# opteroncx/MoePhoto

Measured on AMD Instinct MI355X. Metric: megapixels/sec (input), 1080p 4x SR (Net4x a4), 256-px tiles with overlap, higher is better.
Workload: dtype fp16; 1 GPU; BASELINE configs[1]: 1 frame(s) 1920x1080 RGB -> 7680x4320, model a4 (Net4x, synthetic weights in zoo format), crop 256 pad 5 align 8 -> 40 tiles/frame, fp16 I/O, fp16 MFMA operands + fp32 accumulate; tiles_per_frame=40, parallelism=single GPU, precision=mixed, exact_blocks=1, input=natural-image-like synthetic frame (tests/golden_defs.natural_image)

## Files before the change

moephoto_amd/csrc/common.h:

```cpp
#pragma once
#include <hip/hip_runtime.h>
#include <stdint.h>

typedef _Float16 half_t;
typedef __attribute__((ext_vector_type(2))) _Float16 half2_t;
typedef __attribute__((ext_vector_type(4))) _Float16 half4_t;
typedef __attribute__((ext_vector_type(8))) _Float16 half8_t;
typedef __attribute__((ext_vector_type(4))) float float4_t;
typedef __attribute__((ext_vector_type(16))) float float16_t;

constexpr int kCB = 64;
constexpr int kTileW = 32;
constexpr int kTileH = 8;
constexpr int kFragBytes = 1024;

struct ConvArgs {
    const half_t* in;
    half_t* out;
    const half_t* res;
    const half_t* wpk;
    const float* bias;
    const float* bias_img;
    const half_t* zero;
    half_t* trash;
    half_t* out_lo;
    const half_t* in_lo;
    int plane_w;
    const half_t* side16;
    const float* tail1_w;
    float* tail1_out;
    const half_t* res_lo;
    float* acc32;
    int acc_mode;
    long long w_batch_stride;
    int B, H, W;
    int in_cs, out_cs;
    int r;
    int nchunks;
    int G;
    int px, py;
    float slope;
    float scale;
    const half_t* tail_w;
    float* tplanes;
    int tail_form;
    int tail_split;
    int dbg;
    float* pool; int pool_slabs;
};

struct ConvForm {
    int B = 0, H = 0, W = 0, in_cs = 64, out_cs = 64, r = 1, nchunks = 1, G = 1, py = 1;
    float slope = 1.f, scale = 1.f;
    int acc_mode = 0, dbg = 0, tail_form = 0, tail_split = 0, pool_slabs = 0;
    bool res = false, res_lo = false, in_lo = false, out_lo = false, side16 = false, tail = false, tail1 = false, pool = false, plane_w = false;
};
inline ConvForm conv_form(const ConvArgs& a)
{
    ConvForm c;
    c.B = a.B; c.H = a.H; c.W = a.W; c.in_cs = a.in_cs; c.out_cs = a.out_cs; c.r = a.r; c.nchunks = a.nchunks; c.G = a.G; c.py = a.py;
    c.slope = a.slope; c.scale = a.scale; c.acc_mode = a.acc_mode; c.dbg = a.dbg; c.tail_form = a.tail_form; c.tail_split = a.tail_split; c.pool_slabs = a.pool_slabs;
    c.res = a.res != nullptr; c.res_lo = a.res_lo != nullptr; c.in_lo = a.in_lo != nullptr; c.out_lo = a.out_lo != nullptr; c.side16 = a.side16 != nullptr;
    c.tail = a.tplanes != nullptr; c.tail1 = a.tail1_w != nullptr; c.pool = a.pool != nullptr; c.plane_w = a.plane_w != 0;
    return c;
}

struct TailSumLayout { unsigned S, RA, CA, CO, total; int py, px; };
__host__ __device__ inline TailSumLayout tailsum_layout(int B, int H, int W)
{
    TailSumLayout l;
    l.py = (H + kTileH - 1) / kTileH; l.px = (W + kTileW - 1) / kTileW;
    auto up = [](unsigned long long n) { return (unsigned)((n + 63) / 64 * 64); };
    l.S = 0;
    l.RA = l.S + up(16ull * B * H * W);
    l.CA = l.RA + up(8ull * B * l.py * W);
    l.CO = l.CA + up(8ull * B * H * l.px);
    l.total = l.CO + up(4ull * B * l.py * l.px);
    return l;
}
inline bool tailsum_fits(int B, int H, int W)
{
    const unsigned long long el = 16ull * B * H * W + 8ull * B * ((H + kTileH - 1) / kTileH) * W + 8ull * B * H * ((W + kTileW - 1) / kTileW) + 4ull * B * ((H + kTileH - 1) / kTileH) * ((W + kTileW - 1) / kTileW) + 4 * 64;
    return el * 4 < (1ull << 32) - (1ull << 17);
}

struct Conv1x1Args {
    const half_t* in_hi; const half_t* in_lo;
    half_t* out_hi; half_t* out_lo;
    const half_t* w_hi; const half_t* w_lo;
    const float* bias;
    const float* tail_w; float* tail_out;
    float slope;
    int B, H, W, r, nchunks, out_cs;
    int nks;
};
struct Conv1x1Form { int B, H, W, r, nchunks, out_cs; float slope; bool x3, tail, out_lo; };
bool conv1x1_applicable(const Conv1x1Form& a, int max_groups);
bool launch_conv1x1(const Conv1x1Args& a, int max_groups, hipStream_t s);
hipError_t conv1x1_init();

struct Conv1x1F2Args {
    const half_t* in_hi; const half_t* in_lo;
    const half_t* wa_hi; const half_t* wa_lo;
    const half_t* wb_hi; const half_t* wb_lo;
    const float* bias_a; const float* bias_b;
    const float* tail_w; float* tail_out;
    float slope_a, slope_b;
    int B, H, W;
};
bool conv1x1_f2_applicable(int B, int H, int W, float slope_a, float slope_b, int max_groups);
bool launch_conv1x1_f2(const Conv1x1F2Args& a, int max_groups, hipStream_t s);
hipError_t conv1x1_f2_init();

void launch_conv_mfma(const ConvArgs& a, int taps, int nseg, hipStream_t s);
int conv_mfma_max_groups();
hipError_t conv_mfma_init();
bool conv3x3_sp_applicable(const ConvForm& c);
bool launch_conv3x3_sp(const ConvArgs& a, hipStream_t s);
hipError_t conv3x3_sp_init();
bool conv3x3_rw_applicable(const ConvForm& c);
bool launch_conv3x3_rw(const ConvArgs& a, hipStream_t s);
hipError_t conv3x3_rw_init();

struct Ps4Args {
    const half_t* in;
    const half_t* wpk;
    const float* bias;
    const half_t* tail_w;
    half_t* out;
    float* plane;
    float* apron;
    float slope;
    int B, H, W;
    int split;
};
bool launch_conv3x3_ps4(const Ps4Args& a, int max_groups, hipStream_t s);
bool ps4_applicable(int B, int H, int W);
inline bool ps4_tail_applicable(int B, int H, int W, float slope) { return slope < 1.f && ps4_applicable(B, H, W); }
bool ps4_store_applicable(int B, int H, int W, float slope);
size_t ps4_plane_bytes(int B, int H, int W);
size_t ps4_apron_bytes(int B, int H, int W);
hipError_t conv3x3_ps4_init();
struct TailAddArgs {
    const float* p0; const float* p1;
    const float* a0; const float* a1;
    void* y; int y_dtype; const long long* y_off;
    int B, H, W, px;
    int vec_ok;
};
void launch_tailadd(const TailAddArgs& a, hipStream_t s);

struct Ps9Args {
    const half_t* in;
    const half_t* wpk;
    const float* bias;
    const half_t* tail_w;
    float* plane;
    float* apron;
    float slope;
    int B, H, W;
    int split;
    int xcd_map;
};
bool launch_conv3x3_ps9(const Ps9Args& a, int max_groups, hipStream_t s);
bool ps9_applicable(int B, int H, int W);
inline bool ps9_tail_applicable(int B, int H, int W, float slope) { return slope < 1.f && ps9_applicable(B, H, W); }
size_t ps9_plane_bytes(int B, int H, int W);
size_t ps9_apron_bytes(int B, int H, int W);
hipError_t conv3x3_ps9_init();
struct TailAdd3Args {
    const float* p0; const float* p1;
    const float* a0; const float* a1;
    void* y; int y_dtype; const long long* y_off;
    int B, H, W, px;
    int vec_ok;
};
void launch_tailadd3(const TailAdd3Args& a, hipStream_t s);

struct ArsbArgs {
    const half_t* x_hi; const half_t* x_lo;
    half_t* y_hi; half_t* y_lo;
    const half_t* w1; const half_t* w2;
    const half_t* zero;
    float slope;
    int B, H, W;
    int px, py;
    int cin;
    int drop_lo;
    unsigned long long* trace;
};
bool arsb32c_applicable(int B, int H, int W, float slope, bool x_lo, bool y_lo, int cin);
bool launch_arsb32c(ArsbArgs a, int max_groups, hipStream_t s);
hipError_t arsb32c_init();

struct ConvX3Args {
    const half_t* in_hi; const half_t* in_lo;
    half_t* out_hi; half_t* out_lo;
    const half_t* res_hi; const half_t* res_lo;
    const half_t* w_hi; const half_t* w_lo;
    const half_t* zero;
    float slope;
    int B, H, W;
    int px, py;
    float* pool; int pool_slabs;
    const float* gate;
    const half_t* wq_hi16; const unsigned char* wq_hi8; const unsigned char* wq_lo8;
    int in8, out8;
};
struct ConvX3Form {
    int B = 0, H = 0, W = 0, pool_slabs = 0;
    float slope = 1.f;
    bool res = false, res_lo = false, pool = false, gate = false, in8 = false, out8 = false;
};
inline ConvX3Form conv_x3_form(const ConvX3Args& a)
{
    ConvX3Form c;
    c.B = a.B; c.H = a.H; c.W = a.W; c.pool_slabs = a.pool_slabs; c.slope = a.slope;
    c.res = a.res_hi != nullptr; c.res_lo = a.res_lo != nullptr; c.pool = a.pool != nullptr; c.gate = a.gate != nullptr; c.in8 = a.in8 != 0; c.out8 = a.out8 != 0;
    return c;
}
bool conv64_x3_applicable(const ConvX3Form& c, int max_groups);
bool launch_conv64_x3(ConvX3Args a, int max_groups, hipStream_t s);
hipError_t conv64_x3_init();
bool conv64_q8_applicable(const ConvX3Form& c);
bool launch_conv64_q8(ConvX3Args a, int max_groups, hipStream_t s);
hipError_t conv64_q8_init();
bool conv64_sq_applicable(const ConvX3Form& c, int max_groups);
bool launch_conv64_sq(ConvX3Args a, int max_groups, hipStream_t s);
hipError_t conv64_sq_init();
bool conv64_s_applicable(const ConvForm& c);
bool launch_conv64_s(const ConvArgs& a, int max_groups, hipStream_t s);
hipError_t conv64_s_init();
struct ArsbSqArgs {
    const half_t* x_hi; const unsigned char* x_lo8;
    half_t* y_hi; void* y_lo;
    const half_t* w16[2]; const unsigned char* wh8[2]; const unsigned char* wl8[2];
    float slope;
    int B, H, W, out8;
};
bool arsb_sq_applicable(int B, int H, int W, float slope);
bool launch_arsb_sq(const ArsbSqArgs& a, int max_groups, hipStream_t s);
hipError_t arsb_sq_init();

inline int pooled_groups(long long P, long long items, int max_groups)
{
    long long G = 1;
    if (P <= max_groups) G = P * (max_groups / P);
    else for (long long d = max_groups; d >= 1; --d) if (P % d == 0) { G = d; break; }
    return (int)(G < items ? G : items);
}
inline bool pooled_groups_ok(long long P, long long items, int max_groups)
{
    const long long full = items < max_groups ? items : max_groups;
    return 2ll * pooled_groups(P, items, max_groups) >= full;
}

struct DirectConvArgs {
    const half_t* in; half_t* out; const half_t* res;
    const float* w;
    const float* bias;
    long long w_batch_stride;
    int B, H, W, in_cs, out_cs, cin, cout, k, r;
    float slope, scale;
};
void launch_conv_direct(const DirectConvArgs& a, hipStream_t s);

struct StemArgs {
    const void* x; int x_dtype;
    const long long* x_off;
    long long sB, sH, sW;
    const float* w;
    float slope;
    half_t* out;
    half_t* out_lo;
    int B, H, W, taps;
    int out_lo8;
    const float* w2; half_t* out2; half_t* out2_lo;
};
void launch_stem(const StemArgs& a, hipStream_t s);

struct TailArgs {
    const half_t* in0; const half_t* in1;
    const half_t* w0; const half_t* w1;
    const half_t* in0_lo; const half_t* in1_lo;
    const half_t* w0_lo; const half_t* w1_lo;
    int in1_lo8;
    const void* skip; int skip_dtype;
    const long long* skip_off; long long skip_sB, skip_sH, skip_sW;
    void* y; int y_dtype;
    const long long* y_off;
    int B, H, W, taps;
};
void launch_tail(const TailArgs& a, hipStream_t s);

struct TapSumArgs {
    const float* t0; const float* t1;
    void* y; int y_dtype; const long long* y_off;
    int B, H, W;
    int r;
    int form;
    int vec_ok;
};
void launch_tapsum(const TapSumArgs& a, hipStream_t s);

struct Tail1SumArgs {
    const float* p0; const float* p1;
    int nparts;
    void* y; int y_dtype; const long long* y_off;
    int B, H, W;
    const float* lut; int r; const void* x; const long long* x_off; long long sB, sH, sW;
    int vec_ok;
};
void launch_tail1sum(const Tail1SumArgs& a, hipStream_t s);

void launch_pool_partial(const half_t* in, const half_t* in_lo, float* partial, int B, long long HW, int C, int nslab, hipStream_t s);

struct SednSeArgs {
    const float* partial; int nslab; long long HW;
    const float* w_down;
    const float* w_up;
    const float* trans_pk32;
    half_t* trans_out;
    half_t* trans_out_lo;
    int B, nfrag;
};
void launch_sedn_se(const SednSeArgs& a, hipStream_t s);

struct SednFuseArgs {
    const half_t* x;
    float* partial;
    const float* pooled; int pooled_slabs;
    int pooled_count;
    int nslab, B, H, W;
    const float* w256t;
    const float* w256;
    const float* wt;
    const float* w_down;
    const float* w_up;
    float* gate;
    half_t* weff;
};
void launch_sedn_fuse(const SednFuseArgs& a, hipStream_t s);

struct FrmArgs {
    const float* partial; int nslab; long long HW;
    const float* w0; const float* b0;
    const float* w2; const float* b2;
    const half_t* t; const half_t* x; half_t* out;
    const half_t* t_lo; const half_t* x_lo; half_t* out_lo;
    float* gate;
    int B;
};
void launch_frm(const FrmArgs& a, hipStream_t s);
struct FrmPreArgs {
    const half_t* m; const half_t* m_lo;
    const float* partial; int nslab;
    const float* c2t;
    const float* w0; const float* b0;
    const float* w2; const float* b2;
    float* gate;
    int B, H, W;
};
void launch_frm_pre(const FrmPreArgs& a, hipStream_t s);

struct StitchArgs {
    const float* tiles; const long long* tile_off;
    const int* row_first; const int* row_cnt;
    const int* col_first; const int* col_cnt;
    const int* row_tab; const int* col_tab;
    const float* ramp;
    void* out; int out_dtype;
    int C, out_h, out_w, step_w;
    int row_lo;
    int y0, rows;
};
void launch_stitch(const StitchArgs& a, hipStream_t s);
bool launch_stitch_out(const StitchArgs& a, int canvas_dtype, float quant, hipStream_t s);
struct StitchMix {
    const void* inp; long long sC, sH, sW;
    const void* alpha; long long aH, aW;
    float sf, tf; int blend;
    float quant;
    int inp_vec, alpha_vec;
    long long once_from; int q_once;
};
bool launch_stitch_mix(const StitchArgs& a, StitchMix m, int canvas_dtype, hipStream_t s);
struct YuvEdge {
    int ky[3], ku[3], kv[3];
    unsigned mul_y, base_y; int mul_c, base_c;
    int depth, f16;
};
void launch_stitch_yuv(const StitchArgs& a, const YuvEdge& y, hipStream_t s);
void launch_to_output_yuv(const void* src, int src_dtype, int H, int W, const YuvEdge& y, void* dst, hipStream_t s);

struct BlendTileArgs {
    const void* r; void* canvas; const void* ramp;
    long long r_sC, r_sH, c_sC, c_sH;
    int C, rh, rw;
    int top_sc, left_sc;
    int r0, c0;
    int lt_h, lt_w;
};
void launch_blend_tile(const BlendTileArgs& a, bool f16, hipStream_t s);

struct SymArgs {
    const void* src; void* dst;
    long long sC, sH, sW;
    int C, Hd, Wd;
    int nR, nC, flipR, flipC;
    int src_vec;
    int div; float inv;
};
void launch_sym(SymArgs a, bool f16, bool fold, bool tr, hipStream_t s);

struct WireRec {
    long long tile_off, wire_off;
    int C, th, tw;
    int ra0, ra1, rb0, rb1;
    int ca0, ca1, cb0, cb1;
    int pad_;
};
long long wire_rec_words(const WireRec& r);
void launch_wire(bool pack, float* tiles, unsigned* wire, const WireRec* recs, int n, long long max_elems, hipStream_t s);

void launch_to_float(const void* src, int src_dtype, float inv_or_div, bool divide, int H, int W, int C, void* dst, int dst_dtype, hipStream_t s);
void launch_to_output(const void* src, int src_dtype, int H, int W, int C, float quant, void* dst, int dst_dtype, hipStream_t s);
void launch_resize(const void* src, void* dst, int dtype, int C, int H, int W, int h, int w, int mode, hipStream_t s);
void launch_maxabsdiff(const float* a, const float* b, long long n, unsigned* out, hipStream_t s);
void launch_nhwc_to_nchw_f32(const half_t* in, const half_t* in_lo, float* out, int B, int H, int W, int cs, int C, hipStream_t s);
```

moephoto_amd/csrc/forward.cpp:

```cpp
#include "net.h"

using namespace moe;

namespace moe {

const char* kernel_name(ConvKernel k)
{
    static const char* const names[] = {"no kernel", "conv_direct", "conv1x1", "conv_mfma", "conv3x3_sp", "conv3x3_rw", "conv3x3_ps4 (store form)", "conv3x3_sp (hi + lo residual)",
                                        "conv_mfma (three products)", "conv64_x3", "conv64_q8", "conv64_sq", "conv3x3_sp (three launches)", "conv_mfma (fp32 side buffer)"};
    return names[(int)k];
}

static bool fast_layer(const moe_net& n, const ConvLayer& L) { return L.taps == 9 && L.nseg == 1 && !L.per_plane && n.opt.conv_impl == 2; }

ConvForm Fwd::form(const ConvLayer& L, int H, int W) const
{
    ConvForm c;
    c.B = B; c.H = H; c.W = W; c.in_cs = 64 * L.nseg; c.out_cs = L.r > 1 ? 64 : 64 * L.nchunks; c.r = L.r; c.nchunks = L.nchunks;
    c.py = (H + kTileH - 1) / kTileH;
    const long long items = (long long)B * ((W + kTileW - 1) / kTileW) * c.py;
    const int per_xcd = groups / 8;
    int G = per_xcd >= L.nchunks ? 8 * (per_xcd / L.nchunks) : groups / L.nchunks;
    if (G < 1) G = 1;
    if (G > items) G = (int)items;
    c.G = G;
    c.slope = L.slope; c.scale = L.scale; c.dbg = n.opt.dbg;
    return c;
}

ConvRoute Fwd::route(const std::string& key, const Act& in, const Act& out, const Act* res, int H, int W, const ConvExtra& e) const
{
    ConvRoute r;
    auto take = [&r](ConvKernel k) { r.kernel = k; return r; };
    auto refuse = [&r]() { r.kernel = ConvKernel::none; r.done.ok = false; return r; };
    const ConvLayer& L = n.convs[n.conv_index.at(key)];
    const bool x3 = this->x3 || e.exact;
    const bool res_lo = res && res->has_lo;
    const bool any8 = in.lo8 || out.lo8 || (res && res->lo8);
    if (any8 && !(x3 && use_q8() && q8_capable(L) && !direct)) return refuse();
    if (e.fuse_tail1) r.done.tail1_parts = 2;
    ConvForm& c = r.form;
    c = form(L, H, W);
    if (direct) return take(ConvKernel::direct);
    const int px = (W + kTileW - 1) / kTileW;
    c.res = res != nullptr; c.tail1 = e.fuse_tail1;
    c.tail = e.fuse_tail; c.tail_form = e.fuse_tail ? tail_form : 0; c.tail_split = (e.fuse_tail && mixed && tail_split_for(key)) ? 1 : 0;
    if (e.pool && !x3 && L.r == 1 && L.nchunks == 1 && !res && pooled_groups_ok((long long)c.py, (long long)B * c.py, groups)) {
        c.pool = true; c.pool_slabs = e.pool_slabs;
        c.G = pooled_groups((long long)c.py, (long long)B * c.py, groups);
    }
    const bool fast = fast_layer(n, L);
    if (e.fuse_tail && !(fast && !x3)) return refuse();
    if (n.opt.conv1x1 && L.taps == 1 && L.nseg == 1 && !L.per_plane && !res && L.scale == 1.f && !e.fuse_tail && n.opt.conv_impl == 2 && (!x3 || (in.has_lo && L.has_x3)) &&
        conv1x1_applicable(Conv1x1Form{B, H, W, L.r, L.nchunks, c.out_cs, L.slope, x3, e.fuse_tail1, x3 && out.has_lo}, groups)) {
        if (e.fuse_tail1) r.done.tail1_parts = 1;
        return take(ConvKernel::conv1x1);
    }
    const bool traced = !x3 && (c.dbg & 64) && fast && key == n.opt.trace_key;
    if (!x3 && !traced && res_lo && out.has_lo) {
        c.acc_mode = 3; c.side16 = true; c.out_lo = true;
        r.done.ok = fast && conv3x3_sp_applicable(c);
        return take(ConvKernel::sp_res_lo);
    }
    if (!x3) {
        if (c.tail && c.tail_form == 1) { r.done.ok = conv3x3_rw_applicable(c); return take(ConvKernel::rw); }
        if (fast && n.opt.up_impl == 1 && !c.tail && !c.pool && c.r == 2 && c.nchunks == 4 && c.in_cs == 64 && !c.res && c.scale == 1.f && !c.dbg && L.has_bias &&
            (long long)B * px * (H / 4) >= 32ll * groups && ps4_store_applicable(B, H, W, L.slope))
            return take(ConvKernel::ps4_store);
        if (fast && n.opt.sp_impl && !c.tail && conv3x3_rw_applicable(c)) { r.done.pooled = c.pool; return take(ConvKernel::rw); }
        if (fast && conv3x3_sp_applicable(c)) return take(ConvKernel::sp);
        if (c.tail) return refuse();
        return take(ConvKernel::mfma);
    }
    if (L.has_x3 && !fast) return take(ConvKernel::mfma_x3);
    if (n.opt.x3_fuse && fast && L.w_arsb_lo && in.has_lo && out.has_lo && (!res || res_lo) && !e.fuse_tail && !L.has_bias) {
        ConvX3Form q;
        q.B = B; q.H = H; q.W = W; q.slope = L.slope; q.res = res != nullptr; q.res_lo = res_lo;
        const long long P = (long long)px * c.py;
        if (e.pool && !res && (L.slope == 1.f || e.pool_act) && pooled_groups_ok(P, (long long)B * P, groups)) { q.pool = true; q.pool_slabs = e.pool_slabs; }
        if (e.gate && res && !use_q8()) q.gate = true;
        r.x3 = q;
        if (use_q8() && L.wq_hi8 && !q.pool && (!res || res->lo8 == in.lo8)) {
            r.x3.in8 = in.lo8; r.x3.out8 = out.lo8;
            if (n.opt.q8_impl == 1 && conv64_sq_applicable(r.x3, groups)) return take(ConvKernel::sq);
            if (conv64_q8_applicable(r.x3)) return take(ConvKernel::q8);
            r.x3 = q;
        }
        if (any8) return refuse();
        if (conv64_x3_applicable(q, groups)) { r.done.pooled = q.pool; r.done.gated = q.gate; return take(ConvKernel::x3); }
    }
    if (fast && L.nchunks <= 16) {
        ConvForm q1 = c; q1.res = res_lo; q1.slope = 1.f; q1.scale = 1.f; q1.tail = false;
        ConvForm q2 = q1; q2.res = true;
        ConvForm q3 = c; q3.acc_mode = 3; q3.side16 = true; q3.out_lo = out.has_lo;
        if (conv3x3_sp_applicable(q1) && conv3x3_sp_applicable(q2) && conv3x3_sp_applicable(q3)) return take(ConvKernel::sp_three);
    }
    if (!acc32_elems) return refuse();
    return take(ConvKernel::acc32);
}

int Fwd::launch(const ConvRoute& r, const std::string& key, const Act& in, const Act& out, const Act* res, const ConvExtra& e)
{
    const ConvLayer& L = n.convs[n.conv_index.at(key)];
    const ConvForm& c = r.form;
    const int H = c.H, W = c.W;
    if (r.kernel == ConvKernel::direct) {
        DirectConvArgs d{};
        d.in = in.hi; d.out = out.hi; d.res = res ? res->hi : nullptr;
        d.w = blob<float>(L.w_plain);
        d.bias = L.has_bias ? blob<float>(L.bias_plain) : nullptr;
        d.w_batch_stride = 0;
        d.B = B; d.H = H; d.W = W; d.in_cs = c.in_cs; d.out_cs = c.out_cs; d.cin = L.cin; d.cout = L.cout; d.k = L.k; d.r = L.r;
        d.slope = L.slope; d.scale = L.scale;
        if (L.per_plane) { d.w = (const float*)e.plane_w; d.w_batch_stride = (long long)L.cout * L.cin; }
        launch_conv_direct(d, s);
        return MOE_OK;
    }
    ConvArgs a{};
    a.in = in.hi; a.out = out.hi; a.res = res ? res->hi : nullptr;
    a.wpk = L.per_plane ? e.plane_w : blob<half_t>(L.w_hi);
    a.bias = L.has_bias ? blob<float>(L.bias) : small<float>("zero_bias");
    a.zero = small<half_t>("zero");
    a.bias_img = blob<float>(L.bias_img);
    a.trash = small<half_t>("trash");
    a.w_batch_stride = L.per_plane ? (long long)L.nchunks * L.nfrag() * 512 : 0;
    a.B = B; a.H = H; a.W = W; a.in_cs = c.in_cs; a.out_cs = c.out_cs; a.r = c.r; a.nchunks = c.nchunks;
    a.px = (W + kTileW - 1) / kTileW; a.py = c.py; a.G = c.G;
    a.slope = c.slope; a.scale = c.scale; a.dbg = c.dbg;
    a.tail_w = e.tail_w; a.tplanes = e.tplanes; a.tail_form = c.tail_form; a.tail_split = c.tail_split;
    a.tail1_w = e.tail1_w; a.tail1_out = e.tail1_out;
    if (c.pool) { a.pool = e.pool_out; a.pool_slabs = c.pool_slabs; }
    const bool x3 = this->x3 || e.exact;
    const bool timed = r.kernel != ConvKernel::mfma_x3 && r.kernel != ConvKernel::sp_three && r.kernel != ConvKernel::acc32;
    const int rec = timed ? prof_begin(key, (x3 ? 3 : 1) * 2.0 * (double)B * H * W * L.cout * L.cin * L.taps) : -1;
    bool ok = true;
    auto single = [&](const ConvArgs& ca) {
        if (r.kernel == ConvKernel::rw) return launch_conv3x3_rw(ca, s);
        if (r.kernel == ConvKernel::sp) return launch_conv3x3_sp(ca, s);
        if (r.kernel == ConvKernel::ps4_store) {
            Ps4Args q{};
            q.in = ca.in; q.wpk = ca.wpk; q.bias = ca.bias; q.out = ca.out; q.slope = ca.slope; q.B = ca.B; q.H = ca.H; q.W = ca.W;
            return launch_conv3x3_ps4(q, groups, s);
        }
        launch_conv_mfma(ca, L.taps, L.nseg, s);
        return true;
    };
    switch (r.kernel) {
    case ConvKernel::conv1x1: {
        Conv1x1Args q{};
        q.in_hi = in.hi; q.in_lo = x3 ? in.lo : nullptr; q.out_hi = out.hi; q.out_lo = x3 ? out.lo : nullptr;
        q.w_hi = blob<half_t>(L.w_hi); q.w_lo = x3 ? blob<half_t>(L.w_lo) : nullptr; q.bias = a.bias;
        q.tail_w = e.tail1_w; q.tail_out = e.tail1_out; q.slope = L.slope;
        q.B = B; q.H = H; q.W = W; q.r = L.r; q.nchunks = L.nchunks; q.out_cs = c.out_cs;
        q.nks = (L.cin <= 48 && n.opt.k48) ? 3 : 4;
        ok = launch_conv1x1(q, groups, s);
        break;
    }
    case ConvKernel::mfma: case ConvKernel::sp: case ConvKernel::rw: case ConvKernel::ps4_store: {
        unsigned long long* tr = nullptr;
        const size_t nb = 8 * 32 * 4 * 16 * 8;
        if (!x3 && (c.dbg & 64) && fast_layer(n, L) && key == n.opt.trace_key && hipMalloc((void**)&tr, nb) == hipSuccess) {
            (void)hipMemsetAsync(tr, 0, nb, s);
            ConvArgs t = a; t.acc32 = (float*)tr;
            ok = single(t);
            std::vector<unsigned long long> host(nb / 8);
            (void)hipStreamSynchronize(s);
            (void)hipMemcpy(host.data(), tr, nb, hipMemcpyDeviceToHost);
            if (FILE* f = fopen("/tmp/moe_trace.bin", "wb")) { fwrite(host.data(), 1, nb, f); fclose(f); }
            (void)hipFree(tr);
        } else
            ok = single(a);
        break;
    }
    case ConvKernel::sp_res_lo: {
        ConvArgs q = a; q.acc_mode = 3; q.side16 = res->lo; q.out_lo = out.lo; q.res_lo = nullptr;
        ok = launch_conv3x3_sp(q, s);
        break;
    }
    case ConvKernel::mfma_x3: {
        ConvArgs f4 = a; f4.wpk = blob<half_t>(L.w_x3); f4.acc_mode = 4; f4.in_lo = in.lo; f4.out_lo = out.lo; f4.res_lo = res ? res->lo : nullptr;
        launch_conv_mfma(f4, 1, 3, s);
        break;
    }
    case ConvKernel::x3: case ConvKernel::q8: case ConvKernel::sq: {
        ConvX3Args q{};
        q.in_hi = in.hi; q.in_lo = in.lo; q.out_hi = out.hi; q.out_lo = out.lo;
        q.res_hi = res ? res->hi : nullptr; q.res_lo = res ? res->lo : nullptr;
        q.w_hi = blob<half_t>(L.w_arsb); q.w_lo = blob<half_t>(L.w_arsb_lo); q.zero = small<half_t>("zero");
        q.slope = L.slope; q.B = B; q.H = H; q.W = W;
        if (r.x3.pool) { q.pool = e.pool_out; q.pool_slabs = e.pool_slabs; }
        if (r.x3.gate) q.gate = e.gate_in;
        if (r.kernel == ConvKernel::x3) { ok = launch_conv64_x3(q, groups, s); break; }
        q.wq_hi16 = blob<half_t>(L.w_hi); q.wq_hi8 = blob<unsigned char>(L.wq_hi8); q.wq_lo8 = blob<unsigned char>(L.wq_lo8);
        q.in8 = r.x3.in8; q.out8 = r.x3.out8;
        ok = r.kernel == ConvKernel::sq ? launch_conv64_sq(q, groups, s) : launch_conv64_q8(q, groups, s);
        break;
    }
    case ConvKernel::sp_three: {
        ConvArgs q1 = a; q1.wpk = blob<half_t>(L.w_lo); q1.out = side16; q1.res = (res && res->has_lo) ? res->lo : nullptr; q1.bias = small<float>("zero_bias");
        q1.bias_img = small<float>("zero_bias_img"); q1.slope = 1.f; q1.scale = 1.f; q1.acc_mode = 0; q1.tail_w = nullptr; q1.tplanes = nullptr;
        ConvArgs q2 = q1; q2.in = in.lo; q2.wpk = blob<half_t>(L.w_hi); q2.res = side16;
        ConvArgs q3 = a; q3.acc_mode = 3; q3.side16 = side16; q3.out_lo = out.lo; q3.res_lo = nullptr;
        ok = launch_conv3x3_sp(q1, s) && launch_conv3x3_sp(q2, s) && launch_conv3x3_sp(q3, s);
        break;
    }
    case ConvKernel::acc32: {
        a.acc32 = acc32;
        ConvArgs p1 = a; p1.wpk = L.per_plane ? e.plane_w_lo : blob<half_t>(L.w_lo); p1.acc_mode = 1; p1.res = nullptr; p1.bias = nullptr;
        launch_conv_mfma(p1, L.taps, L.nseg, s);
        ConvArgs p2 = a; p2.in = in.lo; p2.acc_mode = 2; p2.res = nullptr; p2.bias = nullptr;
        launch_conv_mfma(p2, L.taps, L.nseg, s);
        ConvArgs p3 = a; p3.acc_mode = 3; p3.out_lo = out.lo; p3.res_lo = res ? res->lo : nullptr;
        launch_conv_mfma(p3, L.taps, L.nseg, s);
        break;
    }
    default: ok = false;
    }
    prof_end(rec);
    if (!ok) return fail(MOE_EINVAL, "internal error: layer %s (%d planes of %dx%d) was routed to %s, and that launcher refused it", key.c_str(), B, H, W, kernel_name(r.kernel));
    return MOE_OK;
}

ConvDone Fwd::conv(const std::string& key, const Act& in, const Act& out, const Act* res, int H, int W, const ConvExtra& e)
{
    const ConvRoute r = route(key, in, out, res, H, W, e);
    if (r.done.ok && !dry()) {
        rc = launch(r, key, in, out, res, e);
        if (rc) ar.base = nullptr;
    }
    return r.done;
}

void Fwd::stem(const Act& out, const Act* out2)
{
    if (dry()) return;
    StemArgs a{};
    if (out2) { a.w2 = small<float>("stem.p2"); a.out2 = out2->hi; a.out2_lo = out2->lo; }
    a.x = io.x; a.x_dtype = io.x_dtype; a.x_off = io.x_off; a.sB = io.sB; a.sH = io.sH; a.sW = io.sW;
    a.w = small<float>("stem"); a.slope = n.scalars.at("stem_slope");
    a.out = out.hi; a.out_lo = out.lo; a.out_lo8 = out.lo8; a.B = B; a.H = h; a.W = w; a.taps = (int)n.scalars.at("stem_taps");
    launch_stem(a, s);
}

void Fwd::gate() { if (ctx.gate_event && !dry()) (void)hipStreamWaitEvent(s, ctx.gate_event, 0); }

void Fwd::tail(const Act* r, const Act* u, int H, int W, bool skip)
{
    gate();
    if (dry()) return;
    TailArgs a{};
    a.in0 = r->hi; a.w0 = small<half_t>("tail_r");
    if (u) { a.in1 = u->hi; a.w1 = small<half_t>("tail_u"); }
    if (r->has_lo && (!u || u->has_lo)) {
        a.in0_lo = r->lo; a.w0_lo = small<half_t>("tail_r.lo");
        if (u) { a.in1_lo = u->lo; a.w1_lo = small<half_t>("tail_u.lo"); a.in1_lo8 = u->lo8; }
    }
    if (skip) { a.skip = io.x; a.skip_dtype = io.x_dtype; a.skip_off = io.x_off; a.skip_sB = io.sB; a.skip_sH = io.sH; a.skip_sW = io.sW; }
    a.y = io.y; a.y_dtype = io.y_dtype; a.y_off = io.y_off; a.B = B; a.H = H; a.W = W; a.taps = (int)n.scalars.at("tail_taps");
    launch_tail(a, s);
}

static size_t acc32_need(const moe_net& n, int B, int h, int w)
{
    size_t best = 0;
    long long HW = (long long)h * w;
    if (n.arch == MOE_ARCH_SEDN) return (size_t)B * (size_t)HW * 256;
    int rr = 1;
    best = (size_t)B * (size_t)HW * 64;
    for (int s = 0; s < n.stages; ++s) {
        best = std::max<size_t>(best, (size_t)B * (size_t)HW * rr * rr * 64 * n.r * n.r);
        rr *= n.r;
    }
    return best;
}

int exact_blocks_of(const moe_net& n)
{
    if (n.exact_blocks >= 0) return n.exact_blocks > 6 ? 6 : n.exact_blocks;
    const int env = n.opt.exact_blocks_env;
    if (env >= 0) return env > 6 ? 6 : env;
    if (n.calib_valid && n.calib_blocks >= 0) return n.calib_blocks;
    return default_exact_blocks(n.arch);
}

int default_exact_blocks(int arch)
{
    switch (arch) {
        case MOE_ARCH_NET2X: return 4;
        case MOE_ARCH_NET3X: return 2;
        case MOE_ARCH_NET4X: return 1;
        case MOE_ARCH_NETDN: return 1;
        default: return 0;
    }
}

long long sp_bytes_per_pixel(const moe_net& n)
{
    long long per = 128;
    if (n.arch == MOE_ARCH_SEDN) per = 512;
    if (n.arch == MOE_ARCH_LITE) {
        for (int st = 0; st + 1 < n.stages; ++st) per *= 4;
    }
    if (n.arch == MOE_ARCH_NET2X || n.arch == MOE_ARCH_NET3X || n.arch == MOE_ARCH_NET4X) {
        long long rr = 1;
        for (int st = 0; st < n.stages; ++st) {
            rr *= (long long)n.r * n.r;
            per = std::max(per, st == n.stages - 1 ? 36 * rr : 128 * rr);
        }
    }
    return per;
}

static int run_forward(const moe_net& n, Fwd& f, const FwdIO& io)
{
    const int B = f.B, h = f.h, w = f.w;
    const long long P = (long long)B * h * w;
    f.io = io;
    if (f.x3) {
        f.acc32_elems = acc32_need(n, B, h, w);
        f.acc32 = (float*)f.ar.take(f.acc32_elems * 4);
        f.side16 = (half_t*)f.ar.take(f.acc32_elems * 2 + 4096);
    } else if (f.mixed) {
        f.side16 = (half_t*)f.ar.take((size_t)P * 64 * 2 + 4096);
        bool steep = false;
        for (int i = 1; i <= exact_blocks_of(n); ++i) steep = steep || n.convs[n.conv_index.at("c1_" + std::to_string(i))].slope > 1.f;
        if (steep) { f.acc32_elems = (size_t)P * 64; f.acc32 = (float*)f.ar.take(f.acc32_elems * 4); }
    }
    int rc = MOE_OK;
    switch (n.arch) {
        case MOE_ARCH_SEDN: rc = forward_sedn(n, f); break;
        case MOE_ARCH_LITE: rc = forward_lite(n, f); break;
        default: rc = forward_arsb(n, f);
    }
    return rc ? rc : f.rc;
}

static Fwd make_fwd(const moe_net& n, const FwdCtx& ctx, NetRuntime* rt, hipStream_t s, int B, int h, int w, Arena ar)
{
    Fwd f{n, ctx, rt, s, B, h, w, ar, ctx.groups, n.precision == MOE_PREC_FP16X3, n.precision == MOE_PREC_DEBUG_DIRECT};
    f.mixed = n.precision == MOE_PREC_MIXED;
    return f;
}

static size_t workspace_need(const moe_net& n, const FwdCtx& ctx, int B, int h, int w)
{
    Fwd f = make_fwd(n, ctx, nullptr, nullptr, B, h, w, Arena{});
    run_forward(n, f, FwdIO{});
    return f.ar.off + 4096;
}

static bool plan_matches(const Fwd& f, size_t planned)
{
    if (f.ar.overflow) return false;
    return f.skips_planned_work ? f.ar.off <= planned : f.ar.off == planned;
}

static int forward_dev_chunk(moe_net& n, const FwdIO& io, int B, int h, int w, hipStream_t s, bool y_off_mult8, const FwdCtx& ctx);

static void build_lite_lut_on_device(moe_net& n, hipStream_t s, const FwdCtx& ctx)
{
    const int r = n.scale;
    std::vector<unsigned short> pat(65536);
    for (int i = 0; i < 65536; ++i) pat[(size_t)i] = (unsigned short)i;
    half_t* in = nullptr;
    float* scratch = nullptr;
    int rc = MOE_ENOMEM;
    if (hipMalloc((void**)&in, 65536 * 2) == hipSuccess && hipMalloc((void**)&n.lut, (size_t)65536 * r * r * 4) == hipSuccess && hipMalloc((void**)&scratch, (size_t)65536 * r * r * 4) == hipSuccess &&
        hipMemcpyAsync(in, pat.data(), 65536 * 2, hipMemcpyHostToDevice, s) == hipSuccess && hipStreamSynchronize(s) == hipSuccess) {
        FwdCtx capture = ctx;
        capture.lut_capture = n.lut;
        rc = forward_dev_chunk(n, FwdIO{in, MOE_F16, 65536, 256, 1, nullptr, scratch, MOE_F32, nullptr}, 1, 256, 256, s, true, capture);
        (void)hipStreamSynchronize(s);
    }
    if (in) (void)hipFree(in);
    if (scratch) (void)hipFree(scratch);
    if (rc != MOE_OK) { (void)hipGetLastError(); drop_lut(n); }
    n.lut_state = rc == MOE_OK ? 1 : -1;
}

static void build_lite_lut(moe_net& n, hipStream_t s, const FwdCtx& ctx)
{
    n.lut_state = -1;
    if (n.arch != MOE_ARCH_LITE || !n.opt.lite_lut || n.debug || !n.opt.fuse_tail || n.precision == MOE_PREC_DEBUG_DIRECT) return;
    hipStreamCaptureStatus cs = hipStreamCaptureStatusNone;
    if (hipStreamIsCapturing(s, &cs) != hipSuccess || cs != hipStreamCaptureStatusNone) { (void)hipGetLastError(); n.lut_state = 0; return; }
    int cur = -1;
    if (hipGetDevice(&cur) != hipSuccess || (cur != n.device && hipSetDevice(n.device) != hipSuccess)) { (void)hipGetLastError(); n.lut_state = 0; return; }
    build_lite_lut_on_device(n, s, ctx);
    if (cur != n.device) (void)hipSetDevice(cur);
}

int forward_dev(moe_net& n, const FwdIO& io, int B, int h, int w, hipStream_t s, bool y_off_mult8, const FwdCtx& ctx)
{
    if (!n.finalized) return fail(MOE_ESTATE, "moe_net_forward: net is not finalized (load_state_dict + to(device) first)");
    if (B < 1 || h < 1 || w < 1) return fail(MOE_EINVAL, "moe_net_forward: bad shape B=%d h=%d w=%d", B, h, w);
    if ((io.x_dtype != MOE_F32 && io.x_dtype != MOE_F16) || (io.y_dtype != MOE_F32 && io.y_dtype != MOE_F16))
        return fail(MOE_EINVAL, "moe_net_forward: x/y dtype must be MOE_F32 or MOE_F16");
    const long long bmax = kSpRange / (sp_bytes_per_pixel(n) * (long long)h * w);
    if (bmax < 1)
        return fail(MOE_ENOMEM, "a %dx%d tile exceeds the convolution kernels' addressing range (%lld pixels per plane at most for this net): use a smaller cropsize",
                    h, w, kSpRange / sp_bytes_per_pixel(n));
    if (n.arch == MOE_ARCH_LITE && io.x_dtype == MOE_F16 && n.lut_state == 0 && n.opt.lite_lut) build_lite_lut(n, s, ctx);
    if (B <= bmax) return forward_dev_chunk(n, io, B, h, w, s, y_off_mult8, ctx);
    const size_t xe = io.x_dtype == MOE_F32 ? 4 : 2, ye = io.y_dtype == MOE_F32 ? 4 : 2;
    const long long yplane = (long long)h * n.scale * w * n.scale;
    for (int b0 = 0; b0 < B; b0 += (int)bmax) {
        const int cnt = (int)std::min<long long>(bmax, B - b0);
        FwdIO c = io;
        if (io.x_off) c.x_off += b0; else c.x = (const char*)io.x + (size_t)b0 * io.sB * xe;
        if (io.y_off) c.y_off += b0; else c.y = (char*)io.y + (size_t)b0 * yplane * ye;
        const bool al = y_off_mult8 && (io.y_off || ((size_t)b0 * yplane * ye) % 16 == 0);
        if (int rc = forward_dev_chunk(n, c, cnt, h, w, s, al, ctx)) return rc;
    }
    return MOE_OK;
}

static int forward_dev_chunk(moe_net& n, const FwdIO& io, int B, int h, int w, hipStream_t s, bool y_off_mult8, const FwdCtx& ctx)
{
    int cur = -1;
    HIP_TRY(hipGetDevice(&cur));
    if (cur != n.device) HIP_TRY(hipSetDevice(n.device));
    const size_t need = workspace_need(n, ctx, B, h, w);
    StreamSet& set = *ctx.set;
    if (int rc = set.ws.grow(need, s, "workspace of %zu bytes for %d planes of %dx%d does not fit", need, B, h, w)) return rc;
    const size_t planned = need - 4096;
    Fwd f = make_fwd(n, ctx, &n.rt, s, B, h, w, Arena{(char*)set.ws.p, 0, planned});
    f.y_vec = y_off_mult8 && ((uintptr_t)io.y % 16 == 0);
    int rc = run_forward(n, f, io);
    if (rc) return rc;
    if (!plan_matches(f, planned))
        return fail(MOE_EINVAL, "internal error: the launching pass took %zu bytes of workspace%s, the planning pass %zu (%d planes of %dx%d)", f.ar.off,
                    f.ar.overflow ? " (beyond the plan: the launches behind that point were not issued)" : "", planned, B, h, w);
    hipError_t e = hipGetLastError();
    if (e != hipSuccess) return fail(MOE_EHIP, "kernel launch failed: %s", hipGetErrorString(e));
    return MOE_OK;
}

void free_set(StreamSet& set)
{
    if (set.side) { (void)hipStreamSynchronize(set.side); (void)hipStreamDestroy(set.side); }
    for (hipEvent_t e : {set.ev_fork, set.ev_join}) if (e) (void)hipEventDestroy(e);
    set.ws.release();
    set = StreamSet{};
}

void free_records(NetRuntime& rt)
{
    for (auto& ev : rt.prof_ev) { (void)hipEventDestroy(ev.e0); (void)hipEventDestroy(ev.e1); }
    for (auto& sl : rt.off_ring) {
        if (sl.host) (void)hipHostFree(sl.host);
        if (sl.dev) (void)hipFree(sl.dev);
        if (sl.done) (void)hipEventDestroy(sl.done);
    }
    for (auto& t : rt.taps) if (t.second.dev) (void)hipFree(t.second.dev);
    rt = NetRuntime{};
}

void pipe_destroy(moe_net& n)
{
    for (auto& ps : n.pipe) {
        if (ps.main) { (void)hipStreamSynchronize(ps.main); (void)hipStreamDestroy(ps.main); }
        for (hipEvent_t e : {ps.entry, ps.done}) if (e) (void)hipEventDestroy(e);
        free_set(ps);
        ps = PipeSet{};
    }
    n.pipe_prev_valid = false;
    n.pipe_last_stream = nullptr;
}

static bool overlap_eligible(const moe_net& n, int B, int h, int w)
{
    const bool sr = n.arch == MOE_ARCH_NET2X || n.arch == MOE_ARCH_NET3X || n.arch == MOE_ARCH_NET4X;
    return sr && n.finalized && n.opt.overlap_calls && !n.debug && n.opt.conv_impl == 2 && (n.precision == MOE_PREC_MIXED || n.precision == MOE_PREC_FP16) &&
           (long long)B * h * w <= 4ll * 65536 && n.prof_keys.empty() && n.opt.repeat_key.empty();
}

static int forward_pipelined(moe_net* n, const void* x, int x_dtype, int B, int h, int w, int64_t sB, int64_t sH, int64_t sW, void* y, int y_dtype, hipStream_t s, unsigned flags)
{
    HIP_TRY(hipSetDevice(n->device));
    PipeSet& ps = n->pipe[n->pipe_next];
    PipeSet& prev = n->pipe[n->pipe_next ^ 1];
    if (!ps.main) {
        HIP_TRY(hipStreamCreateWithFlags(&ps.main, hipStreamNonBlocking));
        HIP_TRY(hipEventCreateWithFlags(&ps.entry, hipEventDisableTiming));
        HIP_TRY(hipEventCreateWithFlags(&ps.done, hipEventDisableTiming));
    }
    HIP_TRY(hipEventRecord(ps.entry, s));
    const bool since_prev = (flags & MOE_FWD_INPUT_SINCE_PREV) && n->pipe_prev_valid && n->pipe_last_stream == s && prev.entry;
    HIP_TRY(hipStreamWaitEvent(ps.main, since_prev ? prev.entry : ps.entry, 0));
    n->pipe_next ^= 1;
    const int groups = n->opt.overlap_groups > 0 ? std::max(16, std::min(n->opt.overlap_groups, n->max_groups)) : std::max(16, n->max_groups / 2);
    const FwdCtx ctx{&ps, groups, n->opt.overlap_fork && n->opt.branch_streams, since_prev ? ps.entry : nullptr, nullptr};
    const int rc = forward_dev(*n, FwdIO{x, x_dtype, sB, sH, sW, nullptr, y, y_dtype, nullptr}, B, h, w, ps.main, true, ctx);
    if (hipEventRecord(ps.done, ps.main) != hipSuccess || hipStreamWaitEvent(s, ps.done, 0) != hipSuccess) { (void)hipGetLastError(); (void)hipStreamSynchronize(ps.main); }
    n->pipe_prev_valid = rc == MOE_OK;
    n->pipe_last_stream = s;
    return rc;
}

}

extern "C" {

int moe_net_forward_ex(moe_net* n, const void* x, int x_dtype, int B, int h, int w, int64_t sB, int64_t sH, int64_t sW,
                       const int64_t* x_off, void* y, int y_dtype, const int64_t* y_off, void* stream, unsigned flags)
{
    if (!n || !x || !y) return fail(MOE_EINVAL, "moe_net_forward: NULL argument");
    if (flags & ~(unsigned)MOE_FWD_INPUT_SINCE_PREV) return fail(MOE_EINVAL, "moe_net_forward_ex: unknown flags 0x%x", flags);
    if ((flags & MOE_FWD_INPUT_SINCE_PREV) && !x_off && !y_off && B >= 1 && h >= 1 && w >= 1 && overlap_eligible(*n, B, h, w)) {
        hipStreamCaptureStatus cs = hipStreamCaptureStatusNone;
        if (hipStreamIsCapturing((hipStream_t)stream, &cs) == hipSuccess && cs == hipStreamCaptureStatusNone)
            return forward_pipelined(n, x, x_dtype, B, h, w, sB, sH, sW, y, y_dtype, (hipStream_t)stream, flags);
        (void)hipGetLastError();
    }
    n->pipe_prev_valid = false;
    return moe_net_forward(n, x, x_dtype, B, h, w, sB, sH, sW, x_off, y, y_dtype, y_off, stream);
}

int moe_net_forward(moe_net* n, const void* x, int x_dtype, int B, int h, int w, int64_t sB, int64_t sH, int64_t sW,
                    const int64_t* x_off, void* y, int y_dtype, const int64_t* y_off, void* stream)
{
    if (!n || !x || !y) return fail(MOE_EINVAL, "moe_net_forward: NULL argument");
    hipStream_t s = (hipStream_t)stream;
    long long* xo = nullptr;
    long long* yo = nullptr;
    NetRuntime::OffSlot* slot = nullptr;
    if (x_off || y_off) {
        HIP_TRY(hipSetDevice(n->device >= 0 ? n->device : 0));
        NetRuntime::OffSlot& sl = n->rt.off_ring[n->rt.off_next];
        n->rt.off_next = (n->rt.off_next + 1) % 4;
        if (sl.used) HIP_TRY(hipEventSynchronize(sl.done));
        const size_t need = (size_t)B * 2;
        if (need > sl.cap) {
            if (sl.host) { (void)hipHostFree(sl.host); sl.host = nullptr; }
            if (sl.dev) { (void)hipFree(sl.dev); sl.dev = nullptr; }
            sl.cap = 0;
            const size_t cap = std::max<size_t>(need, 256);
            HIP_TRY(hipHostMalloc((void**)&sl.host, cap * 8, hipHostMallocDefault));
            HIP_TRY(hipMalloc((void**)&sl.dev, cap * 8));
            sl.cap = cap;
        }
        if (!sl.done) HIP_TRY(hipEventCreateWithFlags(&sl.done, hipEventDisableTiming));
        for (int i = 0; i < B; ++i) { sl.host[i] = x_off ? x_off[i] : 0; sl.host[B + i] = y_off ? y_off[i] : 0; }
        HIP_TRY(hipMemcpyAsync(sl.dev, sl.host, need * 8, hipMemcpyHostToDevice, s));
        sl.used = true;
        slot = &sl;
        if (x_off) xo = sl.dev;
        if (y_off) yo = sl.dev + B;
    }
    bool mult8 = true;
    if (y_off) for (int i = 0; i < B; ++i) mult8 = mult8 && (y_off[i] % 8 == 0);
    const int rc = forward_dev(*n, FwdIO{x, x_dtype, sB, sH, sW, xo, y, y_dtype, yo}, B, h, w, s, mult8, own_ctx(*n, &n->set));
    if (slot && hipEventRecord(slot->done, s) != hipSuccess) { (void)hipGetLastError(); (void)hipStreamSynchronize(s); }
    return rc;
}

int64_t moe_net_workspace_bytes(const moe_net* n, int B, int h, int w)
{
    if (!n || B < 1 || h < 1 || w < 1) return fail(MOE_EINVAL, "moe_net_workspace_bytes: bad argument");
    if (!n->finalized) return fail(MOE_ESTATE, "moe_net_workspace_bytes: net is not finalized");
    return (int64_t)workspace_need(*n, own_ctx(*n, nullptr), B, h, w);
}

int moe_net_set_profile(moe_net* n, const char* layer_substrings)
{
    if (!n) return fail(MOE_EINVAL, "moe_net_set_profile: NULL net");
    n->prof_keys.clear();
    std::string all = layer_substrings ? layer_substrings : "";
    size_t pos = 0;
    while (pos <= all.size() && !all.empty()) {
        const size_t c = all.find(',', pos);
        const std::string k = all.substr(pos, c == std::string::npos ? std::string::npos : c - pos);
        if (!k.empty()) n->prof_keys.push_back(k);
        if (c == std::string::npos) break;
        pos = c + 1;
    }
    n->rt.prof_used = 0;
    return MOE_OK;
}

int moe_net_get_profile_at(moe_net* n, int index, double* total_ms, int64_t* launches, double* flops)
{
    if (!n || !total_ms || !launches || !flops) return fail(MOE_EINVAL, "moe_net_get_profile: NULL argument");
    double ms = 0, fl = 0;
    int64_t cnt = 0;
    for (size_t i = 0; i < n->rt.prof_used; ++i) {
        const NetRuntime::ProfRec& r = n->rt.prof_ev[i];
        if (r.key != index) continue;
        HIP_TRY(hipEventSynchronize(r.e1));
        float t = 0.f;
        HIP_TRY(hipEventElapsedTime(&t, r.e0, r.e1));
        ms += t; fl += r.flops; ++cnt;
    }
    *total_ms = ms; *launches = cnt; *flops = fl;
    return MOE_OK;
}

int moe_net_get_profile(moe_net* n, double* total_ms, int64_t* launches, double* flops)
{
    int rc = moe_net_get_profile_at(n, 0, total_ms, launches, flops);
    if (rc == MOE_OK) n->rt.prof_used = 0;
    return rc;
}

int64_t moe_net_max_tile_pixels(const moe_net* n)
{
    if (!n) return fail(MOE_EINVAL, "moe_net_max_tile_pixels: NULL net");
    return (int64_t)(kSpRange / sp_bytes_per_pixel(*n));
}

int moe_net_set_debug(moe_net* n, int enable)
{
    if (!n) return fail(MOE_EINVAL, "moe_net_set_debug: NULL net");
    n->debug = enable != 0;
    return MOE_OK;
}

int64_t moe_net_debug_tap(moe_net* n, const char* tap, float* host, int64_t capacity, int64_t shape[4], void* stream)
{
    if (!n || !tap) return fail(MOE_EINVAL, "moe_net_debug_tap: NULL argument");
    auto it = n->rt.taps.find(tap);
    if (it == n->rt.taps.end() || !it->second.dev) return fail(MOE_EINVAL, "no tap named \"%s\" (enable moe_net_set_debug before the forward)", tap);
    const auto& t = it->second;
    const int64_t nel = t.shape[0] * t.shape[1] * t.shape[2] * t.shape[3];
    if (shape) for (int d = 0; d < 4; ++d) shape[d] = t.shape[d];
    if (!host) return nel;
    if (capacity < nel) return fail(MOE_EINVAL, "moe_net_debug_tap: capacity %lld < %lld", (long long)capacity, (long long)nel);
    HIP_TRY(hipStreamSynchronize((hipStream_t)stream));
    HIP_TRY(hipMemcpy(host, t.dev, (size_t)nel * 4, hipMemcpyDeviceToHost));
    return nel;
}

}
```

moephoto_amd/csrc/forward_arsb.cpp:

```cpp
#include "net.h"

using namespace moe;

namespace {

const ConvLayer* last_up(const moe_net& n, int br)
{
    const auto it = n.conv_index.find(std::string(br == 0 ? "convt_R1" : "u") + ".up" + std::to_string(n.stages - 1));
    return it == n.conv_index.end() ? nullptr : &n.convs[it->second];
}

bool can_fuse_tail(const moe_net& n, const Fwd& f)
{
    const int B = f.B, h = f.h, w = f.w;
    if (!n.opt.fuse_tail || f.x3 || f.direct || n.debug || n.opt.conv_impl != 2 || n.stages < 1) return false;
    if (!(n.arch == MOE_ARCH_NET2X || n.arch == MOE_ARCH_NET3X || n.arch == MOE_ARCH_NET4X)) return false;
    if (sp_bytes_per_pixel(n) * B * h * w > kSpRange) return false;
    int hl = h, wl = w;
    for (int st = 0; st + 1 < n.stages; ++st) { hl *= n.r; wl *= n.r; }
    for (int br = 0; br < 2; ++br) {
        const ConvLayer* L = last_up(n, br);
        if (!L) return false;
        ConvForm c = f.form(*L, hl, wl);
        c.tail = true;
        if (!conv3x3_sp_applicable(c)) return false;
    }
    return true;
}

struct ArsbRun {
    const moe_net& n;
    Fwd& f;
    const int B, h, w;
    bool mixed = false;
    int nx = 0;
    Act A, Bb, Cc;
    bool chain8 = false;
    half_t* lo16x = nullptr;
    bool sr = false, fuse = false, ps4 = false, ps9 = false;
    int H = 0, W = 0;
    Act fin[2];
    float* tp[2] = {nullptr, nullptr};
    float* ps_plane[2] = {nullptr, nullptr};
    float* ps_apron[2] = {nullptr, nullptr};

    void plan_tail_form();
    template <typename Args, typename Launch>
    int ps_stage(int br, const std::string& key, const Act& cur, size_t plane_bytes, size_t apron_bytes, const char* name, Launch launch);
    int run_branch(int br, Act cur);
    int trunk_conv(const std::string& key, const Act& in, const Act& out, const Act* res, bool exact);
    int run_trunk();
    template <typename Args, typename Launch> void tail_add(Launch launch);
    int branch_sum();
    int run();
};

void ArsbRun::plan_tail_form()
{
    sr = n.arch != MOE_ARCH_NETDN;
    fuse = sr && can_fuse_tail(n, f);
    if (sr) {
        int hl = h, wl = w;
        for (int st = 0; st + 1 < n.stages; ++st) { hl *= n.r; wl *= n.r; }
        bool ok = fuse && n.opt.tail_form == 1;
        bool ps4_ok = true;
        bool ps9_ok = true;
        for (int br = 0; br < 2; ++br) {
            const ConvLayer* L = last_up(n, br);
            if (ok) {
                ConvForm c = f.form(*L, hl, wl);
                c.tail = true; c.tail_form = 1;
                ok = conv3x3_rw_applicable(c);
            }
            ps4_ok = ps4_ok && L && ps4_tail_applicable(B, hl, wl, L->slope);
            ps9_ok = ps9_ok && L && ps9_tail_applicable(B, hl, wl, L->slope);
        }
        f.tail_form = ok ? 1 : 0;
        ps4 = ok && n.opt.up_impl == 1 && ps4_ok && (2 * wl) % 8 == 0;
        ps9 = fuse && n.opt.up_impl == 1 && n.r == 3 && f.groups >= 3 && ps9_ok;
    }
}

template <typename Args, typename Launch>
int ArsbRun::ps_stage(int br, const std::string& key, const Act& cur, size_t plane_bytes, size_t apron_bytes, const char* name, Launch launch)
{
    ps_plane[br] = (float*)f.ar.take(plane_bytes + 4096);
    ps_apron[br] = (float*)f.ar.take(apron_bytes + 4096);
    if (!f.dry()) {
        const ConvLayer& L = n.convs[n.conv_index.at(key)];
        Args q{};
        q.in = cur.hi; q.wpk = f.blob<half_t>(L.w_hi); q.bias = L.has_bias ? f.blob<float>(L.bias) : f.small<float>("zero_bias");
        q.tail_w = f.small<half_t>(br == 0 ? "tail_r.frag" : "tail_u.frag");
        q.plane = ps_plane[br]; q.apron = ps_apron[br]; q.slope = L.slope; q.B = B; q.H = H; q.W = W;
        q.split = (f.mixed && f.tail_split_for(key)) ? 1 : 0;
        const int rec = f.prof_begin(key, 2.0 * (double)B * H * W * L.cout * L.cin * L.taps);
        bool done = false;
        for (int rep = f.repeats(key); rep > 0; --rep) done = launch(q, f.groups, f.s);
        f.prof_end(rec);
        if (!done) return fail(MOE_EINVAL, "fused tail kernel (%s) rejected layer %s", name, key.c_str());
    }
    H *= n.r; W *= n.r;
    return (int)MOE_OK;
}

int ArsbRun::run_branch(int br, Act cur)
{
    if (f.mixed) { cur.drop_lo(); cur.lo8 = false; }
    H = h; W = w;
    for (int st = 0; st < n.stages; ++st) {
        const std::string key = std::string(br == 0 ? "convt_R1" : "u") + ".up" + std::to_string(st);
        if (ps4 && st == n.stages - 1) {
            if (int rc = ps_stage<Ps4Args>(br, key, cur, ps4_plane_bytes(B, H, W), ps4_apron_bytes(B, H, W), "ps4", launch_conv3x3_ps4)) return rc;
            continue;
        }
        if (ps9 && st == n.stages - 1) {
            if (int rc = ps_stage<Ps9Args>(br, key, cur, ps9_plane_bytes(B, H, W), ps9_apron_bytes(B, H, W), "ps9", launch_conv3x3_ps9)) return rc;
            continue;
        }
        if (fuse && st == n.stages - 1) {
            tp[br] = (float*)f.ar.take(f.tail_form == 1 ? (size_t)tailsum_layout(B, H, W).total * 4 + 4096 : (size_t)9 * B * H * n.r * W * n.r * 4 + 4096);
            ConvExtra tail;
            tail.fuse_tail = true; tail.tail_w = f.small<half_t>(br == 0 ? "tail_r.frag" : "tail_u.frag"); tail.tplanes = tp[br];
            if (!f.conv(key, cur, Act{}, nullptr, H, W, tail))
                return fail(MOE_EINVAL, "fused tail kernel rejected layer %s", key.c_str());
            H *= n.r; W *= n.r;
            continue;
        }
        Act nxt = f.act((long long)B * H * n.r * W * n.r);
        f.conv(key, cur, nxt, nullptr, H, W);
        H *= n.r; W *= n.r;
        f.tap(std::string(br == 0 ? "r" : "u") + ".up" + std::to_string(st), nxt, H, W, 64, 64);
        cur = nxt;
    }
    fin[br] = cur;
    return (int)MOE_OK;
}

int ArsbRun::trunk_conv(const std::string& key, const Act& in, const Act& out, const Act* res, bool exact)
{
    ConvExtra e;
    e.exact = exact;
    if (!f.conv(key, in, out, res, h, w, e))
        return fail(MOE_EINVAL, "layer %s: %d planes of %dx%d exceed the conv kernel's addressing range (use smaller tiles)", key.c_str(), B, h, w);
    return (int)MOE_OK;
}

int ArsbRun::run_trunk()
{
    if (int rc = trunk_conv("input2", A, Bb, nullptr, mixed)) return rc;
    f.tap("input2", Bb, h, w, 64, n.C);
    const bool arsb_fuse = n.opt.arsb_fuse && !f.x3 && !f.direct && n.opt.conv_impl == 2;
    hipStream_t s = f.s;
    Act cur = Bb, oth = Cc;
    for (int i = 1; i <= 6; ++i) {
        const bool ex = mixed && i <= nx;
        const std::string k1 = "c1_" + std::to_string(i), k2 = "c2_" + std::to_string(i);
        const ConvLayer& L1 = n.convs[n.conv_index.at(k1)];
        const ConvLayer& L2 = n.convs[n.conv_index.at(k2)];
        const bool trunk64 = L1.w_arsb != 0;
        const int cin = (L1.cin == 48 && L2.cin == 48 && n.opt.k48) ? 48 : 64;
        if (arsb_fuse && !ex && (!mixed || (cur.has_lo && oth.has_lo)) && trunk64 && arsb32c_applicable(B, h, w, L1.slope, mixed, mixed, cin)) {
            if (!f.dry()) {
                ArsbArgs q{};
                q.x_hi = cur.hi; q.x_lo = mixed ? cur.lo : nullptr; q.y_hi = oth.hi; q.y_lo = mixed ? oth.lo : nullptr;
                q.w1 = f.blob<half_t>(L1.w_hi); q.w2 = f.blob<half_t>(L2.w_hi); q.zero = f.small<half_t>("zero");
                q.slope = L1.slope; q.B = B; q.H = h; q.W = w; q.cin = cin;
                q.drop_lo = (mixed && i == 6 && n.arch != MOE_ARCH_NETDN && !n.debug) ? 1 : 0;
                const bool trace = n.opt.arsb_trace;
                const size_t tb = 8 * 16 * 4 * 40 * 8;
                if (trace && i == 3 && hipMalloc((void**)&q.trace, tb) == hipSuccess) (void)hipMemsetAsync(q.trace, 0, tb, s);
                const int rec = f.prof_begin("arsb" + std::to_string(i), 2.0 * 2.0 * (double)B * h * w * L1.cout * L1.cin * 9);
                bool done = false;
                for (int rep = f.repeats("arsb" + std::to_string(i)); rep > 0; --rep) done = launch_arsb32c(q, f.groups, s);
                f.prof_end(rec);
                if (q.trace) {
                    std::vector<unsigned long long> host(tb / 8);
                    (void)hipStreamSynchronize(s);
                    (void)hipMemcpy(host.data(), q.trace, tb, hipMemcpyDeviceToHost);
                    if (FILE* fp = fopen("/tmp/arsb_trace.bin", "wb")) { fwrite(host.data(), 1, tb, fp); fclose(fp); }
                    (void)hipFree(q.trace);
                }
                if (!done) return fail(MOE_EINVAL, "internal error: arsb32c rejected layer %s its predicate took", k1.c_str());
            }
            std::swap(cur, oth); cur.lo8 = oth.lo8 = false; f.tap("arsb" + std::to_string(i), cur, h, w, 64, n.C);
            continue;
        }
        if (ex && chain8 && n.opt.exact_fuse && n.opt.q8_impl == 1 && cur.lo8 && cur.has_lo && oth.has_lo && L1.wq_hi8 && L2.wq_hi8 && !L1.has_bias && !L2.has_bias && L2.slope == 1.f &&
            arsb_sq_applicable(B, h, w, L1.slope)) {
            if (!f.dry()) {
                ArsbSqArgs q{};
                q.x_hi = cur.hi; q.x_lo8 = (const unsigned char*)cur.lo; q.y_hi = oth.hi; q.y_lo = oth.lo;
                q.w16[0] = f.blob<half_t>(L1.w_hi); q.wh8[0] = f.blob<unsigned char>(L1.wq_hi8); q.wl8[0] = f.blob<unsigned char>(L1.wq_lo8);
                q.w16[1] = f.blob<half_t>(L2.w_hi); q.wh8[1] = f.blob<unsigned char>(L2.wq_hi8); q.wl8[1] = f.blob<unsigned char>(L2.wq_lo8);
                q.slope = L1.slope; q.B = B; q.H = h; q.W = w; q.out8 = i < nx;
                const int rec = f.prof_begin("xpair" + std::to_string(i), 2.0 * 2.0 * 3.0 * (double)B * h * w * L1.cout * L1.cin * 9);
                const bool done = launch_arsb_sq(q, f.groups, s);
                f.prof_end(rec);
                if (!done) return fail(MOE_EINVAL, "internal error: arsb_sq rejected layer %s its predicate took", k1.c_str());
            }
            std::swap(cur, oth);
            cur.lo8 = i < nx;
            oth.lo8 = false;
            f.tap("arsb" + std::to_string(i), cur, h, w, 64, n.C);
            continue;
        }
        Act m = oth;
        if (mixed && !ex) m.drop_lo();
        m.lo8 = ex && chain8;
        Act bin = cur;
        if (mixed && !ex) bin.drop_lo();
        if (int rc = trunk_conv(k1, bin, m, nullptr, ex)) return rc;
        const Act resid = cur;
        if (ex && chain8 && i == nx) { cur.lo = lo16x ? lo16x : A.lo; cur.lo8 = false; }
        if (int rc = trunk_conv(k2, m, cur, &resid, ex)) return rc;
        f.tap("arsb" + std::to_string(i), cur, h, w, 64, n.C);
    }
    Bb = cur;
    return (int)MOE_OK;
}

template <typename Args, typename Launch>
void ArsbRun::tail_add(Launch launch)
{
    if (f.dry()) return;
    Args t{};
    t.p0 = ps_plane[0]; t.p1 = ps_plane[1]; t.a0 = ps_apron[0]; t.a1 = ps_apron[1];
    t.y = f.io.y; t.y_dtype = f.io.y_dtype; t.y_off = f.io.y_off; t.B = B; t.H = H; t.W = W; t.px = (W / n.r + kTileW - 1) / kTileW;
    t.vec_ok = f.y_vec;
    const int rec = f.prof_begin("tailadd", 0.0);
    f.gate();
    launch(t, f.s);
    f.prof_end(rec);
}

int ArsbRun::branch_sum()
{
    if (ps4) { tail_add<TailAddArgs>(launch_tailadd); return MOE_OK; }
    if (ps9) { tail_add<TailAdd3Args>(launch_tailadd3); return MOE_OK; }
    if (fuse) {
        if (!f.dry()) {
            TapSumArgs t{};
            t.t0 = tp[0]; t.t1 = tp[1]; t.y = f.io.y; t.y_dtype = f.io.y_dtype; t.y_off = f.io.y_off; t.B = B; t.H = H; t.W = W; t.r = n.r;
            t.form = f.tail_form;
            t.vec_ok = n.r == 2 && f.y_vec && W % 8 == 0;
            f.gate();
            launch_tapsum(t, f.s);
        }
        return MOE_OK;
    }
    f.tail(&fin[0], &fin[1], H, W, false);
    return MOE_OK;
}

int ArsbRun::run()
{
    const long long P = (long long)B * h * w;
    hipStream_t s = f.s;
    mixed = f.mixed;
    nx = mixed ? exact_blocks_of(n) : 0;
    A = f.act(P, 64, mixed); Bb = f.act(P, 64, mixed); Cc = f.act(P, 64, mixed);
    if (mixed && n.opt.conv_impl != 2)
        return fail(MOE_EINVAL, "precision 'mixed' runs on the fast 3x3 kernels only: conv_impl=v1 (MOE_CONV_IMPL=v1) is a debugging switch for 'fp16' / 'fp16x3'");
    const bool dn = n.arch == MOE_ARCH_NETDN;
    chain8 = mixed && f.use_q8() && n.opt.lo8 && !n.debug && !f.direct && nx >= 1 && A.has_lo && Bb.has_lo && Cc.has_lo;
    if (dn && (int)n.scalars.at("tail_taps") != 9) chain8 = false;
    for (int i = 0; chain8 && i <= nx; ++i)
        for (int j = (i == 0 ? 2 : 1); chain8 && j <= 2; ++j)
            chain8 = f.q8_capable(n.convs[n.conv_index.at(i == 0 ? std::string("input2") : "c" + std::to_string(j) + "_" + std::to_string(i))]);
    lo16x = (dn && chain8) ? (half_t*)f.ar.take((size_t)P * 64 * 2 + 2048) : nullptr;
    A.lo8 = Bb.lo8 = chain8;
    f.stem(A);
    f.tap("stem", A, h, w, 64, n.C);
    plan_tail_form();
    const bool forked = sr && f.ctx.fork && !n.debug && !f.direct && !f.x3 && n.opt.conv_impl == 2 && (long long)B * h * w <= 4ll * 65536;
    struct ForkGuard {
        StreamSet* set; hipStream_t s; bool armed = false;
        ~ForkGuard()
        {
            if (!armed) return;
            if (hipEventRecord(set->ev_join, set->side) != hipSuccess || hipStreamWaitEvent(s, set->ev_join, 0) != hipSuccess) (void)hipStreamSynchronize(set->side);
        }
    } fork_guard{f.ctx.set, s};
    const int all = f.groups;
    int g_side = 0;
    if (forked && all >= 32) {
        g_side = n.opt.branch_groups > 0 ? n.opt.branch_groups : (n.stages >= 2 ? 5 * all / 16 : 3 * all / 16);
        g_side = std::max(8, std::min(g_side, all - 8) / 8 * 8);
    }
    if (forked) {
        if (g_side) f.groups = g_side;
        if (!f.dry()) {
            StreamSet& set = *f.ctx.set;
            if (!set.side) {
                HIP_TRY(hipStreamCreateWithFlags(&set.side, hipStreamNonBlocking));
                HIP_TRY(hipEventCreateWithFlags(&set.ev_fork, hipEventDisableTiming));
                HIP_TRY(hipEventCreateWithFlags(&set.ev_join, hipEventDisableTiming));
            }
            HIP_TRY(hipEventRecord(set.ev_fork, s));
            HIP_TRY(hipStreamWaitEvent(set.side, set.ev_fork, 0));
            f.s = set.side;
            fork_guard.armed = true;
        }
        const int rc = run_branch(1, A);
        if (g_side) f.groups = all - g_side;
        if (!f.dry()) {
            f.s = s;
            if (!rc) HIP_TRY(hipEventRecord(f.ctx.set->ev_join, f.ctx.set->side));
        }
        if (rc) return rc;
    }
    if (int rc = run_trunk()) return rc;
    if (n.arch == MOE_ARCH_NETDN) { f.tail(&Bb, &A, h, w, false); return MOE_OK; }
    if (mixed) { A.drop_lo(); Bb.drop_lo(); A.lo8 = Bb.lo8 = false; }
    if (!forked) { if (int rc = run_branch(0, Bb)) return rc; if (int rc = run_branch(1, A)) return rc; }
    else {
        if (int rc = run_branch(0, Bb)) return rc;
        if (!f.dry()) { HIP_TRY(hipStreamWaitEvent(s, f.ctx.set->ev_join, 0)); fork_guard.armed = false; }
        f.groups = all;
    }
    return branch_sum();
}

}

int moe::forward_arsb(const moe_net& n, Fwd& f)
{
    ArsbRun r{n, f, f.B, f.h, f.w};
    return r.run();
}
```

moephoto_amd/csrc/net.h:

```cpp
#pragma once
#include "engine.h"

#include <algorithm>
#include <cmath>
#include <cstdarg>
#include <cstdio>
#include <cstdlib>
#include <cstring>
#include <map>
#include <memory>
#include <utility>

namespace moe {

int fail(int code, const char* fmt, ...);

#define HIP_TRY(expr)                                                                                    \
    do {                                                                                                 \
        hipError_t e_ = (expr);                                                                          \
        if (e_ != hipSuccess) return fail(e_ == hipErrorOutOfMemory ? MOE_ENOMEM : MOE_EHIP, "%s: %s", #expr, hipGetErrorString(e_)); \
    } while (0)

struct DevBuf {
    void* p = nullptr;
    size_t bytes = 0;
    template <typename... A> int grow(size_t need, hipStream_t s, const char* does_not_fit, A... a)
    {
        if (need <= bytes) return MOE_OK;
        if (p) { HIP_TRY(hipStreamSynchronize(s)); HIP_TRY(hipFree(p)); p = nullptr; bytes = 0; }
        if (hipMalloc(&p, need) != hipSuccess) { (void)hipGetLastError(); p = nullptr; return fail(MOE_ENOMEM, does_not_fit, a...); }
        bytes = need;
        return MOE_OK;
    }
    void release() { if (p) (void)hipFree(p); p = nullptr; bytes = 0; }
};

struct Param {
    std::string name;
    std::vector<int64_t> shape;
    std::vector<float> data;
    bool set = false;
    int64_t numel() const { int64_t n = 1; for (auto d : shape) n *= d; return n; }
};

struct ConvLayer {
    int taps = 9, nseg = 1, nchunks = 1, r = 1;
    int cin = 64, cout = 64, k = 3;
    float slope = 1.f, scale = 1.f;
    bool per_plane = false;
    size_t w_hi = 0, w_lo = 0, bias = 0, bias_img = 0, w_plain = 0, bias_plain = 0, w_pk32 = 0;
    size_t w_arsb_lo = 0;
    size_t wq_hi8 = 0, wq_lo8 = 0;
    size_t w_arsb = 0;
    size_t w_x3 = 0;
    bool has_x3 = false;
    bool has_bias = false;
    int nfrag() const { return nseg * taps * 8; }
};

struct Act {
    half_t* hi = nullptr; half_t* lo = nullptr; bool lo8 = false; bool has_lo = false;
    void drop_lo() { lo = nullptr; has_lo = false; }
};

struct Arena {
    char* base = nullptr;
    size_t off = 0;
    size_t limit = 0;
    bool overflow = false;
    void* take(size_t bytes)
    {
        const size_t a = (off + 255) & ~(size_t)255;
        off = a + bytes;
        if (base && off > limit) { overflow = true; base = nullptr; }
        return base ? base + a : nullptr;
    }
};

struct NetOptions {
    int conv_impl = 2;
    int sp_impl = 1;
    int tail_split = 1;
    int tail_form = 1;
    int up_fuse2 = 1;
    int up_impl = 1;
    int conv1x1 = 1;
    int x3_fuse = 1;
    int arsb_fuse = 1;
    int lo8 = 1;
    int x3_impl = 0;
    int k48 = 1;
    int s64 = 1;
    int branch_streams = 1;
    int branch_groups = 0;
    int exact_fuse = 1;
    int q8_impl = 1;
    int fuse_tail = 1;
    int sedn_fuse = 1;
    int pool_fuse = 1;
    int lite_lut = 1;
    int stem2 = 1;
    int frm_pre = 1;
    int overlap_calls = 1;
    int overlap_fork = 0;
    int overlap_groups = 0;
    int calib_log = 0;
    int auto_calibrate = 1;
    int exact_blocks_env = -1;
    int tiles_per_batch = 0;
    int max_groups = 0;
    int dbg = 0;
    std::string trace_key = "convt_R1.up1";
    bool arsb_trace = false;
    std::string repeat_key;
    int repeat_n = 1;


    bool set(const std::string& key, const char* v);
    void from_env();
};

struct StreamSet { DevBuf ws; hipStream_t side = nullptr; hipEvent_t ev_fork = nullptr, ev_join = nullptr; };
struct PipeSet : StreamSet { hipStream_t main = nullptr; hipEvent_t entry = nullptr, done = nullptr; };

struct NetRuntime {
    struct ProfRec { hipEvent_t e0 = nullptr, e1 = nullptr; int key = 0; double flops = 0; };
    std::vector<ProfRec> prof_ev;
    size_t prof_used = 0;
    struct Tap { float* dev = nullptr; int64_t shape[4] = {0, 0, 0, 0}; };
    std::map<std::string, Tap> taps;
    struct OffSlot { long long* host = nullptr; long long* dev = nullptr; size_t cap = 0; hipEvent_t done = nullptr; bool used = false; };
    OffSlot off_ring[4];
    int off_next = 0;
};

}

struct moe_net {
    int arch = 0, scale = 1;
    moe::NetOptions opt;
    int C = 64;
    int stages = 1, r = 2;
    std::vector<moe::Param> params;
    std::map<std::string, int> index;
    bool finalized = false;
    int device = -1, precision = MOE_PREC_FP16;
    int exact_blocks = -1;
    bool calib_valid = false;
    float* lut = nullptr; int lut_state = 0;
    int calib_blocks = -1;
    double calib_err = 0.0;
    int auto_resolved = -1;
    char* blob = nullptr;
    size_t blob_bytes = 0;
    std::vector<moe::ConvLayer> convs;
    std::map<std::string, int> conv_index;
    std::map<std::string, size_t> small;
    std::map<std::string, float> scalars;
    int max_groups = 256;
    std::vector<std::string> prof_keys;
    bool debug = false;
    moe::StreamSet set;
    moe::PipeSet pipe[2];
    int pipe_next = 0;
    bool pipe_prev_valid = false;
    hipStream_t pipe_last_stream = nullptr;
    moe::NetRuntime rt;
    moe::DevBuf ens_pad, ens_canvas;

    const moe::Param* get(const std::string& n) const
    {
        auto it = index.find(n);
        return it == index.end() ? nullptr : &params[it->second];
    }
    void add(const std::string& n, std::vector<int64_t> shape)
    {
        index[n] = (int)params.size();
        moe::Param p; p.name = n; p.shape = std::move(shape);
        params.push_back(std::move(p));
    }
};

namespace moe {

struct FwdIO {
    const void* x = nullptr; int x_dtype = MOE_F32; long long sB = 0, sH = 0, sW = 0; const long long* x_off = nullptr;
    void* y = nullptr; int y_dtype = MOE_F32; const long long* y_off = nullptr;
};

struct FwdCtx {
    StreamSet* set = nullptr;
    int groups = 0;
    bool fork = false;
    hipEvent_t gate_event = nullptr;
    float* lut_capture = nullptr;
};
inline FwdCtx own_ctx(const moe_net& n, StreamSet* set) { return FwdCtx{set, n.max_groups, n.opt.branch_streams != 0, nullptr, nullptr}; }

struct ConvExtra {
    const half_t* plane_w = nullptr;
    const half_t* plane_w_lo = nullptr;
    const half_t* tail_w = nullptr;
    float* tplanes = nullptr;
    const float* tail1_w = nullptr;
    float* tail1_out = nullptr;
    bool exact = false;
    float* pool_out = nullptr;
    int pool_slabs = 0;
    bool pool_act = false;
    const float* gate_in = nullptr;
    bool fuse_tail = false, fuse_tail1 = false, pool = false, gate = false;
};
struct ConvDone {
    bool ok = true;
    bool pooled = false;
    bool gated = false;
    int tail1_parts = 0;
    explicit operator bool() const { return ok; }
};
enum class ConvKernel {
    none, direct, conv1x1,
    mfma, sp, rw, ps4_store,
    sp_res_lo,
    mfma_x3,
    x3, q8, sq,
    sp_three, acc32,
};
struct ConvRoute {
    ConvKernel kernel = ConvKernel::none;
    ConvDone done;
    ConvForm form;
    ConvX3Form x3;
};
const char* kernel_name(ConvKernel k);

struct Fwd {
    const moe_net& n;
    const FwdCtx& ctx;
    NetRuntime* rt;
    hipStream_t s;
    int B, h, w;
    Arena ar;
    int groups;
    bool x3, direct;
    bool mixed = false;
    bool y_vec = false;
    float* acc32 = nullptr;
    size_t acc32_elems = 0;
    half_t* side16 = nullptr;
    bool dry() const { return ar.base == nullptr; }
    int rc = 0;
    bool skips_planned_work = false;
    int tail_form = 0;
    FwdIO io;

    Act act(long long pixels, int ch = 64, bool want_lo = false)
    {
        Act a;
        a.hi = (half_t*)ar.take((size_t)pixels * ch * 2 + 2048);
        if (x3 || want_lo) { a.lo = (half_t*)ar.take((size_t)pixels * ch * 2 + 2048); a.has_lo = true; }
        return a;
    }
    template <typename T> T* blob(size_t off) const { return (T*)(n.blob + off); }
    template <typename T> T* small(const std::string& k) const { return (T*)(n.blob + n.small.at(k)); }

    void tap(const std::string& name, const Act& a, int H, int W, int cs, int C)
    {
        if (!n.debug || dry()) return;
        auto& t = rt->taps[name];
        if (t.dev) { (void)hipFree(t.dev); t.dev = nullptr; }
        const size_t nel = (size_t)B * C * H * W;
        if (hipMalloc((void**)&t.dev, nel * 4) != hipSuccess) return;
        t.shape[0] = B; t.shape[1] = C; t.shape[2] = H; t.shape[3] = W;
        launch_nhwc_to_nchw_f32(a.hi, a.lo, t.dev, B, H, W, cs, C, s);
    }

    bool tail_split_for(const std::string& key) const
    {
        const int mode = n.opt.tail_split;
        return mode == 2 || (mode == 1 && key.compare(0, 8, "convt_R1") == 0);
    }

    int prof_begin(const std::string& key, double flops)
    {
        for (size_t i = 0; i < n.prof_keys.size(); ++i) {
            if (key.find(n.prof_keys[i]) == std::string::npos) continue;
            if (rt->prof_used == rt->prof_ev.size()) {
                NetRuntime::ProfRec r;
                if (hipEventCreate(&r.e0) != hipSuccess || hipEventCreate(&r.e1) != hipSuccess) return -1;
                rt->prof_ev.push_back(r);
            }
            NetRuntime::ProfRec& r = rt->prof_ev[rt->prof_used];
            r.key = (int)i; r.flops = flops;
            (void)hipEventRecord(r.e0, s);
            return (int)rt->prof_used++;
        }
        return -1;
    }
    void prof_end(int rec) { if (rec >= 0) (void)hipEventRecord(rt->prof_ev[rec].e1, s); }
    int repeats(const std::string& key) const { return (!n.opt.repeat_key.empty() && key.find(n.opt.repeat_key) != std::string::npos) ? n.opt.repeat_n : 1; }

    bool use_q8() const { return mixed && (n.opt.x3_impl == 2 || (n.opt.x3_impl == 0 && (n.scale > 1 || n.arch == MOE_ARCH_NETDN))); }
    bool q8_capable(const ConvLayer& L) const
    {
        ConvX3Form c;
        c.B = B; c.H = h; c.W = w; c.slope = L.slope; c.in8 = c.out8 = true;
        return n.opt.x3_fuse && n.opt.conv_impl == 2 && L.k == 3 && L.r == 1 && L.nchunks == 1 && L.nseg == 1 && !L.per_plane && L.wq_hi8 && L.w_arsb_lo && !L.has_bias && conv64_q8_applicable(c);
    }

    ConvDone conv(const std::string& key, const Act& in, const Act& out, const Act* res, int H, int W, const ConvExtra& extra = ConvExtra{});
    ConvRoute route(const std::string& key, const Act& in, const Act& out, const Act* res, int H, int W, const ConvExtra& extra = ConvExtra{}) const;
    ConvForm form(const ConvLayer& L, int H, int W) const;
    int launch(const ConvRoute& r, const std::string& key, const Act& in, const Act& out, const Act* res, const ConvExtra& extra);
    void stem(const Act& out, const Act* out2 = nullptr);
    void tail(const Act* r, const Act* u, int H, int W, bool skip);
    void gate();
};

int forward_arsb(const moe_net& n, Fwd& f);
int forward_sedn(const moe_net& n, Fwd& f);
int forward_lite(const moe_net& n, Fwd& f);

int exact_blocks_of(const moe_net& n);
int default_exact_blocks(int arch);
long long sp_bytes_per_pixel(const moe_net& n);
constexpr long long kSpRange = (1ll << 32) - (1ll << 16);
int forward_dev(moe_net& n, const FwdIO& io, int B, int h, int w, hipStream_t s, bool y_off_mult8, const FwdCtx& ctx);
void free_set(StreamSet& set);
void pipe_destroy(moe_net& n);
void free_records(NetRuntime& rt);
inline void free_ens_scratch(moe_net& n) { n.ens_pad.release(); n.ens_canvas.release(); }
int build_device_weights(moe_net& n, int precision);
void drop_lut(moe_net& n);
bool calibratable(const moe_net& n);
int calibrate_blocks(moe_net& n, double target, hipStream_t s);
int calibrate_sedn(moe_net& n, double target, hipStream_t s, bool adopt);

}
```

moephoto_amd/csrc/options.cpp:

```cpp
#include "net.h"

using namespace moe;

namespace {

enum OptionKind {
    kFlag,
    kWords,
    kCount,
    kInt,
    kText,
    kRepeat,
};
struct OptionWord { const char* word; int value; };
struct OptionRow {
    const char* key;
    const char* env;
    OptionKind kind;
    int NetOptions::*num;
    std::string NetOptions::*text;
    OptionWord words[3];
};
constexpr OptionWord kOnOff[] = {{"0", 0}, {"off", 0}, {"1", 1}, {"on", 1}};

const OptionRow kOptionTable[] = {
    {"conv_impl", "MOE_CONV_IMPL", kWords, &NetOptions::conv_impl, nullptr, {{"sp", 2}, {"v1", 0}}},
    {"sp_impl", "MOE_SP_IMPL", kWords, &NetOptions::sp_impl, nullptr, {{"sp", 0}, {"auto", 1}, {"rw", 2}}},
    {"tail_split", "MOE_TAIL_SPLIT", kWords, &NetOptions::tail_split, nullptr, {{"0", 0}, {"r", 1}, {"ru", 2}}},
    {"tail_form", "MOE_TAIL_FORM", kWords, &NetOptions::tail_form, nullptr, {{"planes", 0}, {"sums", 1}}},
    {"up_impl", "MOE_UP_IMPL", kWords, &NetOptions::up_impl, nullptr, {{"rw", 0}, {"ps4", 1}}},
    {"up_fuse2", "MOE_UP_FUSE2", kFlag, &NetOptions::up_fuse2},
    {"conv1x1", "MOE_CONV1X1", kFlag, &NetOptions::conv1x1},
    {"q8_impl", "MOE_Q8_IMPL", kWords, &NetOptions::q8_impl, nullptr, {{"s", 1}, {"p", 0}}},
    {"exact_fuse", "MOE_EXACT_FUSE", kFlag, &NetOptions::exact_fuse},
    {"branch_streams", "MOE_BRANCH_STREAMS", kFlag, &NetOptions::branch_streams},
    {"branch_groups", "MOE_BRANCH_GROUPS", kCount, &NetOptions::branch_groups},
    {"auto_calibrate", "MOE_AUTO_CALIBRATE", kFlag, &NetOptions::auto_calibrate},
    {"overlap_calls", "MOE_OVERLAP_CALLS", kFlag, &NetOptions::overlap_calls},
    {"overlap_groups", "MOE_OVERLAP_GROUPS", kCount, &NetOptions::overlap_groups},
    {"overlap_fork", "MOE_OVERLAP_FORK", kFlag, &NetOptions::overlap_fork},
    {"s64", "MOE_S64", kFlag, &NetOptions::s64},
    {"k48", "MOE_K48", kFlag, &NetOptions::k48},
    {"x3_impl", "MOE_X3_IMPL", kWords, &NetOptions::x3_impl, nullptr, {{"auto", 0}, {"x3", 1}, {"q8", 2}}},
    {"lo8", "MOE_LO8", kFlag, &NetOptions::lo8},
    {"x3_fuse", "MOE_X3_FUSE", kFlag, &NetOptions::x3_fuse},
    {"arsb_fuse", "MOE_ARSB_FUSE", kFlag, &NetOptions::arsb_fuse},
    {"fuse_tail", "MOE_FUSE_TAIL", kFlag, &NetOptions::fuse_tail},
    {"sedn_fuse", "MOE_SEDN_FUSE", kFlag, &NetOptions::sedn_fuse},
    {"pool_fuse", "MOE_POOL_FUSE", kFlag, &NetOptions::pool_fuse},
    {"frm_pre", "MOE_FRM_PRE", kFlag, &NetOptions::frm_pre},
    {"stem2", "MOE_STEM2", kFlag, &NetOptions::stem2},
    {"lite_lut", "MOE_LITE_LUT", kFlag, &NetOptions::lite_lut},
    {"dbg", "MOE_DBG", kInt, &NetOptions::dbg},
    {"trace_key", "MOE_TRACE_KEY", kText, nullptr, &NetOptions::trace_key},
    {"tiles_per_batch", "MOE_TILES_PER_BATCH", kCount, &NetOptions::tiles_per_batch},
    {"max_groups", "MOE_MAX_GROUPS", kCount, &NetOptions::max_groups},
    {"calib_log", nullptr, kFlag, &NetOptions::calib_log},
    {"repeat", nullptr, kRepeat},
};

bool word_value(const OptionWord* words, size_t n, const char* v, int& out)
{
    for (size_t i = 0; i < n; ++i)
        if (words[i].word && !strcmp(v, words[i].word)) { out = words[i].value; return true; }
    return false;
}

}

bool NetOptions::set(const std::string& key, const char* v)
{
    if (!v) return false;
    for (const OptionRow& r : kOptionTable) {
        if (key != r.key) continue;
        int t = 0;
        switch (r.kind) {
            case kFlag: if (!word_value(kOnOff, 4, v, t)) return false; break;
            case kWords: if (!word_value(r.words, 3, v, t)) return false; break;
            case kCount: if ((t = atoi(v)) < 0) return false; break;
            case kInt: t = atoi(v); break;
            case kText: this->*r.text = v; return true;
            case kRepeat: {
                const char* c = strrchr(v, ':');
                if (!c) {
                    if (*v && strcmp(v, "0")) return false;
                    repeat_key.clear(); repeat_n = 1;
                    return true;
                }
                const int cnt = atoi(c + 1);
                if (cnt < 1 || c == v) return false;
                repeat_key.assign(v, c - v); repeat_n = cnt;
                return true;
            }
        }
        this->*r.num = t;
        return true;
    }
    return false;
}

void NetOptions::from_env()
{
    for (const OptionRow& r : kOptionTable)
        if (const char* e = r.env ? getenv(r.env) : nullptr)
            if (!set(r.key, e)) fprintf(stderr, "moephoto_amd: %s=\"%s\" is not a value of option %s -- ignored\n", r.env, e, r.key);

    if (const char* e = getenv("MOE_EXACT_BLOCKS")) exact_blocks_env = atoi(e);
    arsb_trace = getenv("MOE_ARSB_TRACE") != nullptr;
}

extern "C" int moe_net_set_option(moe_net* n, const char* key, const char* value)
{
    if (!n || !key || !value) return fail(MOE_EINVAL, "moe_net_set_option: NULL argument");
    if (!n->opt.set(key, value)) return fail(MOE_EINVAL, "moe_net_set_option: unknown option or value \"%s\" = \"%s\"", key, value);
    drop_lut(*n);
    if (!strcmp(key, "max_groups") && n->finalized) n->max_groups = n->opt.max_groups > 0 ? n->opt.max_groups : conv_mfma_max_groups();
    return MOE_OK;
}
```

moephoto_amd/csrc/plan_run.cpp:

```cpp
#include "net.h"

using namespace moe;

static int launched(const char* who)
{
    hipError_t e = hipGetLastError();
    if (e != hipSuccess) return fail(MOE_EHIP, "%s launch failed: %s", who, hipGetErrorString(e));
    return MOE_OK;
}

struct TileTable {
    int device = -1, n_frames = 0;
    int64_t sC = 0, sH = 0, sW = 0, frame_stride = 0;
    std::vector<int64_t> tile_dst;
    bool y_mult8 = false;
    std::vector<int> group_first, group_count;
    void* dev = nullptr;
    const long long *x_off = nullptr, *y_off = nullptr;
};

struct StitchTables {
    int device = -1, C = 0;
    void* dev = nullptr;
    long long* tile_off = nullptr;
    int *row_first = nullptr, *row_cnt = nullptr, *col_first = nullptr, *col_cnt = nullptr, *row_tab = nullptr, *col_tab = nullptr;
    float* ramp = nullptr;
    std::vector<std::pair<int, int*>> strip_tabs;
};

struct UploadedOffsets { int device; std::vector<int64_t> host; void* dev; };

struct PlanDevice {
    static constexpr size_t kCached = 16;
    std::vector<TileTable> tables;
    std::vector<StitchTables> stitch;
    std::vector<UploadedOffsets> uploaded;
    DevBuf pool;
    ~PlanDevice()
    {
        for (auto& t : tables) (void)hipFree(t.dev);
        for (auto& t : stitch) { (void)hipFree(t.dev); for (auto& e : t.strip_tabs) (void)hipFree(e.second); }
        for (auto& u : uploaded) (void)hipFree(u.dev);
        pool.release();
    }
    template <typename V> static int make_room(V& v, hipStream_t s)
    {
        if (v.size() < kCached) return MOE_OK;
        HIP_TRY(hipStreamSynchronize(s));
        (void)hipFree(v.front().dev);
        v.erase(v.begin());
        return MOE_OK;
    }
};

static int upload(const void* host, size_t bytes, void** dev)
{
    HIP_TRY(hipMalloc(dev, bytes));
    const hipError_t e = hipMemcpy(*dev, host, bytes, hipMemcpyHostToDevice);
    if (e != hipSuccess) { (void)hipFree(*dev); *dev = nullptr; }
    HIP_TRY(e);
    return MOE_OK;
}

struct moe_plan { Plan p; mutable PlanDevice dev; };

static int tile_table(const moe_plan& pl, int device, int64_t frame_stride, int64_t sC, int64_t sH, int64_t sW, int n_frames, const int64_t* tile_dst,
                      hipStream_t s, const TileTable** out)
{
    const Plan& p = pl.p;
    const size_t n = p.tiles.size() * (size_t)n_frames;
    for (const TileTable& c : pl.dev.tables)
        if (c.device == device && c.sC == sC && c.sH == sH && c.sW == sW && c.frame_stride == frame_stride && c.n_frames == n_frames &&
            std::equal(c.tile_dst.begin(), c.tile_dst.end(), tile_dst)) { *out = &c; return MOE_OK; }
    int rc = PlanDevice::make_room(pl.dev.tables, s);
    if (rc) return rc;
    TileTable d;
    std::vector<long long> off, yo;
    int slot = 0;
    for (const auto& g : p.groups) {
        d.group_first.push_back(slot);
        const long long plane = (long long)(g.th * p.sc) * (g.tw * p.sc);
        for (int f = 0; f < n_frames; ++f)
            for (int k : g.tiles) {
                const long long at = tile_dst[(size_t)f * p.tiles.size() + k];
                if (at < 0) continue;
                const TileRect& t = p.tiles[k];
                for (int c = 0; c < p.C; ++c) {
                    off.push_back((long long)f * frame_stride + (long long)c * sC + (long long)t.top * sH + (long long)t.left * sW);
                    yo.push_back(at + (long long)c * plane);
                }
                ++slot;
            }
        d.group_count.push_back(slot - d.group_first.back());
    }
    if (off.empty()) { off.push_back(0); yo.push_back(0); }
    d.y_mult8 = true;
    for (long long v : yo) d.y_mult8 = d.y_mult8 && (v % 8 == 0);
    off.insert(off.end(), yo.begin(), yo.end());
    rc = upload(off.data(), off.size() * 8, &d.dev);
    if (rc) return rc;
    d.x_off = (const long long*)d.dev; d.y_off = d.x_off + yo.size();
    d.device = device; d.sC = sC; d.sH = sH; d.sW = sW; d.frame_stride = frame_stride; d.n_frames = n_frames;
    d.tile_dst.assign(tile_dst, tile_dst + n);
    pl.dev.tables.push_back(std::move(d));
    *out = &pl.dev.tables.back();
    return MOE_OK;
}

static int run_sets(moe_net& n, const Plan& p, const TileTable& d, const void* img, int img_dtype, int64_t sH, int64_t sW, float* dst, int max_tiles, hipStream_t s)
{
    if (max_tiles <= 0) {
        max_tiles = n.opt.tiles_per_batch > 0 ? n.opt.tiles_per_batch : 32;
    }
    for (size_t gi = 0; gi < p.groups.size(); ++gi) {
        const auto& g = p.groups[gi];
        const int nt = d.group_count[gi];
        if (nt < 1) continue;
        const long long px = (long long)g.th * g.tw;
        const int per = (int)std::max<long long>(1, std::min<long long>(nt, (long long)max_tiles * 65536 / std::max<long long>(px, 1)));
        for (int t0 = 0; t0 < nt; t0 += per) {
            const int cnt = std::min(per, nt - t0);
            const long long slot = (long long)(d.group_first[gi] + t0) * p.C;
            int rc = forward_dev(n, FwdIO{img, img_dtype, 0, sH, sW, d.x_off + slot, dst, MOE_F32, d.y_off + slot}, cnt * p.C, g.th, g.tw, s, d.y_mult8, own_ctx(n, &n.set));
            if (rc) return rc;
        }
    }
    return MOE_OK;
}

static int stitch_tables(const moe_plan& pl, int device, int C, StitchTables** out)
{
    for (StitchTables& c : pl.dev.stitch)
        if (c.device == device && c.C == C) { *out = &c; return MOE_OK; }
    const Plan& p = pl.p;
    std::vector<long long> toff(p.tiles.size());
    for (size_t k = 0; k < toff.size(); ++k) toff[k] = p.tile_off[k] / p.C * C;
    std::vector<char> host;
    auto put = [&](const void* src, size_t bytes) { const size_t a = (host.size() + 255) & ~(size_t)255; host.resize(a + bytes); memcpy(host.data() + a, src, bytes); return a; };
    const size_t o_t = put(toff.data(), toff.size() * 8);
    const size_t o_rf = put(p.row_first.data(), p.row_first.size() * 4), o_rc = put(p.row_cnt.data(), p.row_cnt.size() * 4);
    const size_t o_cf = put(p.col_first.data(), p.col_first.size() * 4), o_cc = put(p.col_cnt.data(), p.col_cnt.size() * 4);
    const size_t o_rt = put(p.row_tab.data(), p.row_tab.size() * 4), o_ct = put(p.col_tab.data(), p.col_tab.size() * 4);
    const float zero = 0.f;
    const size_t o_rp = put(p.ramp.empty() ? &zero : p.ramp.data(), std::max<size_t>(4, p.ramp.size() * 4));
    StitchTables d;
    int rc = upload(host.data(), host.size(), &d.dev);
    if (rc) return rc;
    char* b = (char*)d.dev;
    d.device = device; d.C = C; d.tile_off = (long long*)(b + o_t);
    d.row_first = (int*)(b + o_rf); d.row_cnt = (int*)(b + o_rc); d.col_first = (int*)(b + o_cf); d.col_cnt = (int*)(b + o_cc);
    d.row_tab = (int*)(b + o_rt); d.col_tab = (int*)(b + o_ct); d.ramp = (float*)(b + o_rp);
    pl.dev.stitch.push_back(std::move(d));
    *out = &pl.dev.stitch.back();
    return MOE_OK;
}

struct OutEdge { int canvas_dtype; float quant; const StitchMix* mix = nullptr; const YuvEdge* yuv = nullptr; };
static int stitch(const moe_plan& pl, int device, const float* tiles, const int64_t* tile_off, bool off_on_host, int C, void* out, int out_dtype, const int* band, hipStream_t s,
                  const OutEdge* edge = nullptr)
{
    const Plan& p = pl.p;
    HIP_TRY(hipSetDevice(device));
    StitchTables* d = nullptr;
    int rc = stitch_tables(pl, device, C, &d);
    if (rc) return rc;
    const long long* toff = tile_off ? (const long long*)tile_off : d->tile_off;
    if (tile_off && off_on_host) {
        const size_t nt = p.tiles.size();
        toff = nullptr;
        for (auto& c : pl.dev.uploaded)
            if (c.device == device && std::equal(c.host.begin(), c.host.end(), tile_off)) { toff = (const long long*)c.dev; break; }
        if (!toff) {
            void* up = nullptr;
            rc = PlanDevice::make_room(pl.dev.uploaded, s);
            if (!rc) rc = upload(tile_off, nt * 8, &up);
            if (rc) return rc;
            pl.dev.uploaded.push_back(UploadedOffsets{device, std::vector<int64_t>(tile_off, tile_off + nt), up});
            toff = (const long long*)up;
        }
    }
    StitchArgs a{};
    a.tiles = tiles; a.tile_off = toff;
    a.row_first = d->row_first; a.row_cnt = d->row_cnt; a.col_first = d->col_first; a.col_cnt = d->col_cnt;
    a.row_tab = d->row_tab; a.col_tab = d->col_tab; a.ramp = d->ramp;
    a.out = out; a.out_dtype = out_dtype; a.C = C; a.out_h = p.out_h; a.out_w = p.out_w; a.step_w = p.aw.step;
    a.y0 = 0; a.rows = p.out_h; a.row_lo = 0;
    if (band) {
        const int row0 = band[0], row1 = band[1], nrow = p.ah.step;
        a.row_lo = row0;
        a.y0 = p.row_tab[row0 * 4 + 1];
        a.rows = (row1 < nrow ? p.row_tab[row1 * 4 + 1] : p.out_h) - a.y0;
        if (band[2] && row1 < nrow) {
            int* tab = nullptr;
            for (auto& e : d->strip_tabs) if (e.first == row1) tab = e.second;
            if (!tab) {
                std::vector<int> rt(p.row_tab);
                rt[row1 * 4 + 2] = rt[row1 * 4 + 0];
                rt[row1 * 4 + 3] = rt[row1 * 4 + 1] - rt[row1 * 4 + 0];
                rc = upload(rt.data(), rt.size() * 4, (void**)&tab);
                if (rc) return rc;
                d->strip_tabs.push_back({row1, tab});
            }
            a.row_tab = tab;
        }
    }
    if (edge && edge->yuv) {
        launch_stitch_yuv(a, *edge->yuv, s);
        return launched("stitch_yuv");
    }
    if (edge && edge->mix) {
        if (!launch_stitch_mix(a, *edge->mix, edge->canvas_dtype, s)) return fail(MOE_EINVAL, "moe_stitch_mix: %d planes (1 to 4 are supported)", C + (edge->mix->alpha ? 1 : 0));
        return launched("stitch_mix");
    }
    if (edge) {
        if (!launch_stitch_out(a, edge->canvas_dtype, edge->quant, s)) return fail(MOE_EINVAL, "moe_stitch_out: %d planes (1 to 4 are supported)", C);
        return launched("stitch_out");
    }
    launch_stitch(a, s);
    return launched("stitch");
}

static int out_edge_args(const char* who, int planes, int canvas_dtype, int bits, const void* dst, int dst_dtype)
{
    if (!dst) return fail(MOE_EINVAL, "%s: NULL argument", who);
    if (planes < 1 || planes > 4) return fail(MOE_EINVAL, "%s: %d planes (1 to 4 are supported)", who, planes);
    if (canvas_dtype != MOE_F32 && canvas_dtype != MOE_F16) return fail(MOE_EINVAL, "%s: canvas dtype must be MOE_F32 or MOE_F16", who);
    if (bits != 8 && bits != 16) return fail(MOE_EINVAL, "%s: %d bits (8 or 16)", who, bits);
    if (dst_dtype != MOE_U8 && dst_dtype != MOE_U16) return fail(MOE_EINVAL, "%s: dst dtype must be MOE_U8 or MOE_U16", who);
    if (dst_dtype == MOE_U8 && bits > 8) return fail(MOE_EINVAL, "%s: %d bits do not fit MOE_U8", who, bits);
    return MOE_OK;
}

static int yuv_edge_args(const char* who, int planes, int dtype, int depth, int matrix, int order, const void* dst, YuvEdge* y)
{
    static const int tab[3][3][3] = {{{3483, 11718, 1183}, {-1877, -6315, 8192}, {8192, -7441, -751}},
                                     {{4899, 9617, 1868}, {-2765, -5427, 8192}, {8192, -6860, -1332}},
                                     {{4304, 11108, 972}, {-2288, -5904, 8192}, {8192, -7533, -659}}};
    if (!dst) return fail(MOE_EINVAL, "%s: NULL argument", who);
    if (planes != 3) return fail(MOE_EINVAL, "%s: the plan has %d planes (C must be 3)", who, planes);
    if (dtype != MOE_F32 && dtype != MOE_F16) return fail(MOE_EINVAL, "%s: canvas dtype must be MOE_F32 or MOE_F16", who);
    if (depth != 8 && depth != 10 && depth != 12 && depth != 16) return fail(MOE_EINVAL, "%s: depth %d (8, 10, 12 or 16)", who, depth);
    if (matrix < MOE_YUV_BT709 || matrix > MOE_YUV_BT2020NC) return fail(MOE_EINVAL, "%s: unknown matrix %d", who, matrix);
    if (order != MOE_ORDER_BGR && order != MOE_ORDER_RGB) return fail(MOE_EINVAL, "%s: unknown order %d", who, order);
    for (int p = 0; p < 3; ++p) {
        const int colour = order == MOE_ORDER_BGR ? 2 - p : p;
        y->ky[p] = tab[matrix][0][colour]; y->ku[p] = tab[matrix][1][colour]; y->kv[p] = tab[matrix][2][colour];
    }
    y->mul_y = 219u << (depth - 6); y->base_y = 16u << (depth - 8);
    y->mul_c = 224 << (depth - 8); y->base_c = 128 << (depth - 8);
    y->depth = depth; y->f16 = dtype == MOE_F16;
    return MOE_OK;
}

static int mix_edge_args(const char* who, const Plan& p, int planes, const void* inp, int inp_dtype, int64_t sC, int64_t sH, int64_t sW, const void* alpha, int64_t aH, int64_t aW,
                         double strength, int bits, const void* dst, int dst_dtype, StitchMix* m)
{
    if (!inp || !dst) return fail(MOE_EINVAL, "%s: NULL argument", who);
    if (p.sc != 1) return fail(MOE_EINVAL, "%s: plan scale %d (the blend with the input needs a plan of scale 1)", who, p.sc);
    if (bits != 0 && bits != 8 && bits != 16) return fail(MOE_EINVAL, "%s: %d bits (0 = the canvas, 8 or 16)", who, bits);
    if (inp_dtype != MOE_F32 && inp_dtype != MOE_F16) return fail(MOE_EINVAL, "%s: canvas dtype (the input's) must be MOE_F32 or MOE_F16", who);
    if (bits == 0 && dst_dtype != inp_dtype) return fail(MOE_EINVAL, "%s: dst dtype must be the input's for the canvas form (bits = 0)", who);
    if (bits != 0 && dst_dtype != MOE_U8 && dst_dtype != MOE_U16) return fail(MOE_EINVAL, "%s: dst dtype must be MOE_U8 or MOE_U16 for %d bits", who, bits);
    if (bits > 8 && dst_dtype == MOE_U8) return fail(MOE_EINVAL, "%s: %d bits do not fit MOE_U8", who, bits);
    if (planes < 1 || planes + (alpha ? 1 : 0) > 4) return fail(MOE_EINVAL, "%s: %d planes%s (1 to 4 in all are supported)", who, planes, alpha ? " + alpha" : "");
    if (!std::isfinite(strength)) return fail(MOE_EINVAL, "%s: strength must be finite", who);
    *m = StitchMix{inp, sC, sH, sW, alpha, aH, aW, (float)strength, (float)(1.0 - strength), strength != 1.0, bits ? (float)(1 << bits) : 0.f, 0, 0, 0, 0};
    return MOE_OK;
}

static int run_plan(const char* who, moe_net* n, const moe_plan* pl, const void* img, int img_dtype, int64_t sC, int64_t sH, int64_t sW,
                    void* out, int out_dtype, int max_tiles, float* pool, int shard_index, int shard_count, int do_stitch, void* stream, const OutEdge* edge)
{
    if (!n || !pl || !img || (do_stitch && !out)) return fail(MOE_EINVAL, "%s: NULL argument", who);
    if (!n->finalized) return fail(MOE_ESTATE, "%s: net is not finalized", who);
    const Plan& p = pl->p;
    if (p.sc != n->scale) return fail(MOE_EINVAL, "%s: plan scale %d != net scale %d", who, p.sc, n->scale);
    if (shard_count < 1) { shard_count = 1; shard_index = 0; }
    if (shard_index < 0 || shard_index >= shard_count) return fail(MOE_EINVAL, "%s: shard %d of %d", who, shard_index, shard_count);
    hipStream_t s = (hipStream_t)stream;
    HIP_TRY(hipSetDevice(n->device));
    std::vector<int64_t> at(p.tile_off.begin(), p.tile_off.end());
    for (size_t k = 0; k < at.size(); ++k) if ((int)(k % shard_count) != shard_index) at[k] = -1;
    const TileTable* d = nullptr;
    int rc = tile_table(*pl, n->device, 0, sC, sH, sW, 1, at.data(), s, &d);
    if (rc) return rc;
    if (!pool) {
        rc = pl->dev.pool.grow(p.pool_elems_per_plane_set * 4, s, "tile pool of %zu bytes does not fit", p.pool_elems_per_plane_set * 4);
        if (rc) return rc;
        pool = (float*)pl->dev.pool.p;
    }
    rc = run_sets(*n, p, *d, img, img_dtype, sH, sW, pool, max_tiles, s);
    if (rc || !do_stitch) return rc;
    return stitch(*pl, n->device, pool, nullptr, false, p.C, out, out_dtype, nullptr, s, edge);
}

extern "C" {

int moe_plan_create(const int64_t shape[3], double ram, double ram_coef, int pad, int scale, int align, int cropsize, moe_plan** out)
{
    if (!shape || !out) return fail(MOE_EINVAL, "moe_plan_create: NULL argument");
    auto p = std::make_unique<moe_plan>();
    std::string err;
    int rc = build_plan(p->p, shape, ram, ram_coef, pad, scale, align, cropsize, err);
    if (rc) return fail(rc, "%s", err.c_str());
    *out = p.release();
    return MOE_OK;
}

void moe_plan_destroy(moe_plan* p)
{
    delete p;
}

int moe_plan_info(const moe_plan* p, int64_t info[12])
{
    if (!p || !info) return fail(MOE_EINVAL, "moe_plan_info: NULL argument");
    const Plan& q = p->p;
    const int64_t v[12] = {(int64_t)q.tiles.size(), q.ah.step, q.aw.step, q.out_h, q.out_w, q.pad_h_to, q.pad_w_to, q.pad_sc,
                           q.tile_h, q.tile_w, q.ah.clip, q.aw.clip};
    memcpy(info, v, sizeof v);
    return MOE_OK;
}

int moe_plan_rows(const moe_plan* p, int32_t* rows)
{
    if (!p || !rows) return fail(MOE_EINVAL, "moe_plan_rows: NULL argument");
    memcpy(rows, p->p.row_tab.data(), p->p.row_tab.size() * 4);
    return MOE_OK;
}

static void axis_seams(const std::vector<int>& tab, int i, int out[4])
{
    const int n = (int)tab.size() / 4;
    const int o = tab[i * 4 + 2], ext = tab[i * 4 + 3];
    std::vector<std::pair<int, int>> iv;
    for (int k = 0; k < n; ++k) {
        const int a = std::max(tab[k * 4 + 0] - o, 0), b = std::min(tab[k * 4 + 1] - o, ext);
        if (b > a) iv.push_back({a, b});
    }
    std::sort(iv.begin(), iv.end());
    std::vector<std::pair<int, int>> m;
    for (auto& v : iv) {
        if (!m.empty() && v.first <= m.back().second) m.back().second = std::max(m.back().second, v.second);
        else m.push_back(v);
    }
    while (m.size() > 2) { m[1].second = m.back().second; m.pop_back(); }
    out[0] = out[1] = out[2] = out[3] = 0;
    if (m.size() >= 1) { out[0] = m[0].first; out[1] = m[0].second; out[2] = out[3] = m[0].second; }
    if (m.size() == 2) { out[2] = m[1].first; out[3] = m[1].second; }
}

int moe_plan_seams(const moe_plan* p, int32_t* seams)
{
    if (!p || !seams) return fail(MOE_EINVAL, "moe_plan_seams: NULL argument");
    const Plan& q = p->p;
    for (int i = 0; i < q.ah.step; ++i)
        for (int j = 0; j < q.aw.step; ++j) {
            int r[4], c[4];
            axis_seams(q.row_tab, i, r);
            axis_seams(q.col_tab, j, c);
            int32_t* o = seams + ((size_t)i * q.aw.step + j) * 8;
            for (int e = 0; e < 4; ++e) { o[e] = r[e]; o[4 + e] = c[e]; }
        }
    return MOE_OK;
}

static_assert(sizeof(moe_wire_rec) == sizeof(WireRec) && sizeof(WireRec) == 64, "moe_wire_rec layout");

int64_t moe_wire_words(const moe_wire_rec* rec)
{
    if (!rec) return -1;
    WireRec r;
    memcpy(&r, rec, sizeof r);
    return wire_rec_words(r);
}

static int wire_call(bool pack, float* tiles, void* wire, const moe_wire_rec* recs_dev, int n, int64_t max_elems, void* stream)
{
    if (n < 0 || (n > 0 && (!tiles || !wire || !recs_dev))) return fail(MOE_EINVAL, "moe_wire_%s: bad argument", pack ? "pack" : "unpack");
    launch_wire(pack, tiles, (unsigned*)wire, (const WireRec*)recs_dev, n, max_elems, (hipStream_t)stream);
    return launched("wire kernel");
}

int moe_wire_pack(const float* tiles_dev, void* wire_dev, const moe_wire_rec* recs_dev, int n, int64_t max_elems, void* stream)
{
    return wire_call(true, (float*)tiles_dev, wire_dev, recs_dev, n, max_elems, stream);
}

int moe_wire_unpack(float* tiles_dev, const void* wire_dev, const moe_wire_rec* recs_dev, int n, int64_t max_elems, void* stream)
{
    return wire_call(false, tiles_dev, (void*)wire_dev, recs_dev, n, max_elems, stream);
}

int moe_plan_tiles(const moe_plan* p, int32_t* tiles)
{
    if (!p || !tiles) return fail(MOE_EINVAL, "moe_plan_tiles: NULL argument");
    for (size_t k = 0; k < p->p.tiles.size(); ++k) {
        const TileRect& t = p->p.tiles[k];
        const int32_t v[8] = {t.top, t.bottom, t.left, t.right, t.top_t, t.left_t, t.bsc, t.rsc};
        memcpy(tiles + k * 8, v, sizeof v);
    }
    return MOE_OK;
}

int moe_plan_ramp(const moe_plan* p, float* ramp)
{
    if (!p || !ramp) return fail(MOE_EINVAL, "moe_plan_ramp: NULL argument");
    memcpy(ramp, p->p.ramp.data(), p->p.ramp.size() * 4);
    return MOE_OK;
}

int64_t moe_plan_pool_elems(const moe_plan* p, int C)
{
    if (!p || C < 1) return fail(MOE_EINVAL, "moe_plan_pool_elems: bad argument");
    return (int64_t)(p->p.pool_elems_per_plane_set / p->p.C * C);
}

int moe_plan_tile_offsets(const moe_plan* p, int C, int64_t* off)
{
    if (!p || !off || C < 1) return fail(MOE_EINVAL, "moe_plan_tile_offsets: bad argument");
    for (size_t k = 0; k < p->p.tiles.size(); ++k) off[k] = p->p.tile_off[k] / p->p.C * C;
    return MOE_OK;
}

int moe_stitch(const moe_plan* p, int device, const float* tiles_dev, const int64_t* tile_off, int C, void* out, int out_dtype, void* stream)
{
    if (!p || !tiles_dev || !out || C < 1) return fail(MOE_EINVAL, "moe_stitch: bad argument");
    return stitch(*p, device, tiles_dev, tile_off, true, C, out, out_dtype, nullptr, (hipStream_t)stream);
}

int moe_stitch_dev(const moe_plan* p, int device, const float* tiles_dev, const int64_t* tile_off_dev, int C, void* out, int out_dtype, void* stream)
{
    if (!p || !tiles_dev || !tile_off_dev || !out || C < 1) return fail(MOE_EINVAL, "moe_stitch_dev: bad argument");
    return stitch(*p, device, tiles_dev, tile_off_dev, false, C, out, out_dtype, nullptr, (hipStream_t)stream);
}

int moe_stitch_band(const moe_plan* p, int device, const float* tiles_dev, const int64_t* tile_off_dev, int C, void* out, int out_dtype,
                    int row0, int row1, int strip, void* stream)
{
    if (!p || !tiles_dev || !tile_off_dev || !out || C < 1) return fail(MOE_EINVAL, "moe_stitch_band: bad argument");
    const int nrow = p->p.ah.step;
    if (row0 < 0 || row1 <= row0 || row1 > nrow) return fail(MOE_EINVAL, "moe_stitch_band: tile rows [%d, %d) of %d", row0, row1, nrow);
    const int band[3] = {row0, row1, strip};
    return stitch(*p, device, tiles_dev, tile_off_dev, false, C, out, out_dtype, band, (hipStream_t)stream);
}

int moe_stitch_out(const moe_plan* p, int device, const float* tiles_dev, const int64_t* tile_off_dev, int C, int canvas_dtype, int bits, void* dst, int dst_dtype, void* stream)
{
    if (!p || !tiles_dev || C < 1) return fail(MOE_EINVAL, "moe_stitch_out: bad argument");
    const int rc = out_edge_args("moe_stitch_out", C, canvas_dtype, bits, dst, dst_dtype);
    if (rc) return rc;
    const OutEdge edge{canvas_dtype, (float)(1 << bits)};
    return stitch(*p, device, tiles_dev, tile_off_dev, false, C, dst, dst_dtype, nullptr, (hipStream_t)stream, &edge);
}

int moe_stitch_mix(const moe_plan* p, int device, const float* tiles_dev, const int64_t* tile_off_dev, int C, const void* inp, int inp_dtype, int64_t sC, int64_t sH, int64_t sW,
                   const void* alpha, int64_t aH, int64_t aW, double strength, int bits, void* dst, int dst_dtype, void* stream)
{
    if (!p || !tiles_dev) return fail(MOE_EINVAL, "moe_stitch_mix: NULL argument");
    StitchMix m{};
    const int rc = mix_edge_args("moe_stitch_mix", p->p, C, inp, inp_dtype, sC, sH, sW, alpha, aH, aW, strength, bits, dst, dst_dtype, &m);
    if (rc) return rc;
    const OutEdge edge{inp_dtype, m.quant, &m};
    return stitch(*p, device, tiles_dev, tile_off_dev, false, C, dst, dst_dtype, nullptr, (hipStream_t)stream, &edge);
}

int moe_stitch_yuv(const moe_plan* p, int device, const float* tiles_dev, const int64_t* tile_off_dev, int canvas_dtype, int depth, int matrix, int order, void* dst, void* stream)
{
    if (!p || !tiles_dev) return fail(MOE_EINVAL, "moe_stitch_yuv: NULL argument");
    YuvEdge y{};
    const int rc = yuv_edge_args("moe_stitch_yuv", p->p.C, canvas_dtype, depth, matrix, order, dst, &y);
    if (rc) return rc;
    OutEdge edge{canvas_dtype, 0.f};
    edge.yuv = &y;
    return stitch(*p, device, tiles_dev, tile_off_dev, false, 3, dst, depth == 8 ? MOE_U8 : MOE_U16, nullptr, (hipStream_t)stream, &edge);
}

int moe_blend_tile(const void* r, int64_t r_sC, int64_t r_sH, void* canvas, int64_t c_sC, int64_t c_sH, int dtype, int C,
                   int top_sc, int left_sc, int bsc, int rsc, int topT, int leftT, int pad_sc, const void* ramp, void* stream)
{
    if (!r || !canvas || C < 1) return fail(MOE_EINVAL, "moe_blend_tile: NULL argument");
    if (dtype != MOE_F32 && dtype != MOE_F16) return fail(MOE_EINVAL, "moe_blend_tile: dtype must be MOE_F32 or MOE_F16");
    const int rh = bsc - top_sc, rw = rsc - left_sc;
    if (rh < 1 || rw < 1 || top_sc < 0 || left_sc < 0 || pad_sc < 0) return fail(MOE_EINVAL, "moe_blend_tile: empty or negative window (%d..%d, %d..%d)", top_sc, bsc, left_sc, rsc);
    auto band = [&](int lt, int l, int& first, int& solid) {
        if (lt < 0) lt += l;
        if (lt < 1) { first = solid = 0; return true; }
        first = lt - pad_sc; solid = lt;
        return first >= 0 && lt <= l;
    };
    BlendTileArgs a{};
    if (!band(topT, rh, a.r0, a.lt_h) || !band(leftT, rw, a.c0, a.lt_w))
        return fail(MOE_EINVAL, "moe_blend_tile: blend band outside the window (topT %d, leftT %d, pad_sc %d, window %d x %d)", topT, leftT, pad_sc, rh, rw);
    if ((a.lt_h > a.r0 || a.lt_w > a.c0) && !ramp) return fail(MOE_EINVAL, "moe_blend_tile: ramp is NULL");
    a.r = r; a.canvas = canvas; a.ramp = ramp; a.r_sC = r_sC; a.r_sH = r_sH; a.c_sC = c_sC; a.c_sH = c_sH;
    a.C = C; a.rh = rh; a.rw = rw; a.top_sc = top_sc; a.left_sc = left_sc;
    launch_blend_tile(a, dtype == MOE_F16, (hipStream_t)stream);
    return launched("blend");
}

int moe_run_plan_ex(moe_net* n, const moe_plan* pl, const void* img, int img_dtype, int64_t sC, int64_t sH, int64_t sW,
                    void* out, int out_dtype, int max_tiles, float* pool, int shard_index, int shard_count, int do_stitch, void* stream)
{
    return run_plan("moe_run_plan", n, pl, img, img_dtype, sC, sH, sW, out, out_dtype, max_tiles, pool, shard_index, shard_count, do_stitch, stream, nullptr);
}

int moe_run_plan_out(moe_net* n, const moe_plan* pl, const void* img, int img_dtype, int64_t sC, int64_t sH, int64_t sW,
                     int canvas_dtype, int bits, void* dst, int dst_dtype, int max_tiles, void* stream)
{
    if (!n || !pl || !img) return fail(MOE_EINVAL, "moe_run_plan_out: NULL argument");
    const int rc = out_edge_args("moe_run_plan_out", pl->p.C, canvas_dtype, bits, dst, dst_dtype);
    if (rc) return rc;
    const OutEdge edge{canvas_dtype, (float)(1 << bits)};
    return run_plan("moe_run_plan_out", n, pl, img, img_dtype, sC, sH, sW, dst, dst_dtype, max_tiles, nullptr, 0, 1, 1, stream, &edge);
}

int moe_run_plan_yuv(moe_net* n, const moe_plan* pl, const void* img, int img_dtype, int64_t sC, int64_t sH, int64_t sW,
                     int canvas_dtype, int depth, int matrix, int order, void* dst, int max_tiles, void* stream)
{
    if (!n || !pl || !img) return fail(MOE_EINVAL, "moe_run_plan_yuv: NULL argument");
    YuvEdge y{};
    const int rc = yuv_edge_args("moe_run_plan_yuv", pl->p.C, canvas_dtype, depth, matrix, order, dst, &y);
    if (rc) return rc;
    OutEdge edge{canvas_dtype, 0.f};
    edge.yuv = &y;
    return run_plan("moe_run_plan_yuv", n, pl, img, img_dtype, sC, sH, sW, dst, depth == 8 ? MOE_U8 : MOE_U16, max_tiles, nullptr, 0, 1, 1, stream, &edge);
}

int moe_run_plan_filter(moe_net* n, const moe_plan* pl, const void* img, int img_dtype, int64_t sC, int64_t sH, int64_t sW, const void* alpha, int64_t aH, int64_t aW,
                        double strength, int bits, void* dst, int dst_dtype, int max_tiles, void* stream)
{
    if (!n || !pl || !img) return fail(MOE_EINVAL, "moe_run_plan_filter: NULL argument");
    StitchMix m{};
    const int rc = mix_edge_args("moe_run_plan_filter", pl->p, pl->p.C, img, img_dtype, sC, sH, sW, alpha, aH, aW, strength, bits, dst, dst_dtype, &m);
    if (rc) return rc;
    const OutEdge edge{img_dtype, m.quant, &m};
    return run_plan("moe_run_plan_filter", n, pl, img, img_dtype, sC, sH, sW, dst, dst_dtype, max_tiles, nullptr, 0, 1, 1, stream, &edge);
}

int moe_run_plan_tiles(moe_net* n, const moe_plan* pl, const void* imgs, int img_dtype, int64_t frame_stride,
                       int64_t sC, int64_t sH, int64_t sW, int n_frames, float* dst, const int64_t* tile_dst,
                       int max_tiles, void* stream)
{
    if (!n || !pl || !imgs || !dst || !tile_dst || n_frames < 1) return fail(MOE_EINVAL, "moe_run_plan_tiles: bad argument");
    if (!n->finalized) return fail(MOE_ESTATE, "moe_run_plan_tiles: net is not finalized");
    const Plan& p = pl->p;
    if (p.sc != n->scale) return fail(MOE_EINVAL, "moe_run_plan_tiles: plan scale %d != net scale %d", p.sc, n->scale);
    hipStream_t s = (hipStream_t)stream;
    HIP_TRY(hipSetDevice(n->device));
    const TileTable* d = nullptr;
    int rc = tile_table(*pl, n->device, frame_stride, sC, sH, sW, n_frames, tile_dst, s, &d);
    if (rc) return rc;
    return run_sets(*n, p, *d, imgs, img_dtype, sH, sW, dst, max_tiles, s);
}

int moe_run_plan_frames(moe_net* n, const moe_plan* pl, const void* imgs, int img_dtype, int64_t frame_stride,
                        int64_t sC, int64_t sH, int64_t sW, int n_frames, float* pools, int64_t pool_stride,
                        int owner_index, int owner_count, int max_tiles, void* stream)
{
    if (!n || !pl || !imgs || !pools || n_frames < 1) return fail(MOE_EINVAL, "moe_run_plan_frames: bad argument");
    const Plan& p = pl->p;
    if (owner_count < 1) { owner_count = 1; owner_index = 0; }
    if (owner_index < 0 || owner_index >= owner_count) return fail(MOE_EINVAL, "moe_run_plan_frames: owner %d of %d", owner_index, owner_count);
    if (pool_stride < (int64_t)p.pool_elems_per_plane_set) return fail(MOE_EINVAL, "moe_run_plan_frames: pool stride smaller than one frame's pool");
    const long long nt = (long long)p.tiles.size();
    std::vector<int64_t> at((size_t)(nt * n_frames));
    for (int f = 0; f < n_frames; ++f)
        for (long long k = 0; k < nt; ++k)
            at[(size_t)(f * nt + k)] = ((f * nt + k) % owner_count == owner_index) ? (int64_t)f * pool_stride + p.tile_off[(size_t)k] : -1;
    return moe_run_plan_tiles(n, pl, imgs, img_dtype, frame_stride, sC, sH, sW, n_frames, pools, at.data(), max_tiles, stream);
}

int moe_run_plan(moe_net* n, const moe_plan* pl, const void* img, int img_dtype, int64_t sC, int64_t sH, int64_t sW,
                 void* out, int out_dtype, int max_tiles, void* stream)
{
    return moe_run_plan_ex(n, pl, img, img_dtype, sC, sH, sW, out, out_dtype, max_tiles, nullptr, 0, 1, 1, stream);
}

struct Sym { int t, fh, fv; };
static Sym sym_of(int s)
{
    static const Sym tab[7] = {{1, 0, 0}, {0, 1, 0}, {0, 1, 1}, {1, 0, 1}, {1, 1, 0}, {0, 0, 1}, {1, 1, 1}};
    return s < 0 ? Sym{0, 0, 0} : tab[s];
}

static int sym_pad(const void* src, bool f16, int C, int H, int W, int64_t sC, int64_t sH, int64_t sW, int s, void* dst, int Hp, int Wp, hipStream_t st)
{
    const Sym y = sym_of(s);
    SymArgs a{};
    a.src = src; a.dst = dst; a.sC = sC; a.sH = sH; a.sW = sW; a.C = C; a.Hd = Hp; a.Wd = Wp;
    a.nR = y.t ? W : H; a.nC = y.t ? H : W; a.flipR = y.fv; a.flipC = y.fh;
    launch_sym(a, f16, false, y.t != 0, st);
    return launched("moe_sym_pad");
}

static int sym_fold(void* acc, const void* t, bool f16, int C, int H, int W, int s, int final_div, hipStream_t st)
{
    const Sym y = sym_of(s);
    const int Wt = y.t ? H : W;
    SymArgs a{};
    a.src = t; a.dst = acc; a.sC = (long long)H * W; a.sH = Wt; a.sW = 1; a.C = C; a.Hd = H; a.Wd = W;
    a.nR = H; a.nC = W;
    a.flipR = y.t ? y.fh : y.fv; a.flipC = y.t ? y.fv : y.fh;
    a.div = final_div > 1; a.inv = 1.0f / (float)(final_div > 1 ? final_div : 1);
    launch_sym(a, f16, true, y.t != 0, st);
    return launched("moe_sym_fold");
}

static bool sym_dtype(int dtype) { return dtype == MOE_F32 || dtype == MOE_F16; }

int moe_sym_pad(const void* src, int dtype, int C, int H, int W, int64_t sC, int64_t sH, int64_t sW, int sym, void* dst, int Hp, int Wp, int device, void* stream)
{
    if (!src || !dst) return fail(MOE_EINVAL, "moe_sym_pad: NULL argument");
    if (!sym_dtype(dtype)) return fail(MOE_EINVAL, "moe_sym_pad: dtype must be MOE_F32 or MOE_F16");
    if (sym < 0 || sym > 6) return fail(MOE_EINVAL, "moe_sym_pad: sym %d is not one of the seven symmetries 0..6", sym);
    if (C < 1 || H < 1 || W < 1) return fail(MOE_EINVAL, "moe_sym_pad: size %d x %d x %d must be positive", C, H, W);
    const Sym y = sym_of(sym);
    const int Ht = y.t ? W : H, Wt = y.t ? H : W;
    if (Hp < Ht || Wp < Wt) return fail(MOE_EINVAL, "moe_sym_pad: padded size %d x %d is smaller than the transformed image %d x %d", Hp, Wp, Ht, Wt);
    HIP_TRY(hipSetDevice(device));
    return sym_pad(src, dtype == MOE_F16, C, H, W, sC, sH, sW, sym, dst, Hp, Wp, (hipStream_t)stream);
}

int moe_sym_fold(void* acc, const void* t, int dtype, int C, int H, int W, int sym, int final_div, int device, void* stream)
{
    if (!acc || !t) return fail(MOE_EINVAL, "moe_sym_fold: NULL argument");
    if (!sym_dtype(dtype)) return fail(MOE_EINVAL, "moe_sym_fold: dtype must be MOE_F32 or MOE_F16");
    if (sym < 0 || sym > 6) return fail(MOE_EINVAL, "moe_sym_fold: sym %d is not one of the seven symmetries 0..6", sym);
    if (C < 1 || H < 1 || W < 1) return fail(MOE_EINVAL, "moe_sym_fold: size %d x %d x %d must be positive", C, H, W);
    if (final_div < 0) return fail(MOE_EINVAL, "moe_sym_fold: final_div %d is negative (0 or 1: no division)", final_div);
    HIP_TRY(hipSetDevice(device));
    return sym_fold(acc, t, dtype == MOE_F16, C, H, W, sym, final_div, (hipStream_t)stream);
}

}

static int run_plan_ens(moe_net* n, const moe_plan* pl, const moe_plan* pl_t, int n_sym, const void* img, int img_dtype, int64_t sC, int64_t sH, int64_t sW,
                        void* out, int out_dtype, int max_tiles, hipStream_t s)
{
    const Plan& p = pl->p;
    const bool f16_in = img_dtype == MOE_F16, f16_out = out_dtype == MOE_F16;
    const size_t es_in = f16_in ? 2 : 4, es_out = f16_out ? 2 : 4;
    auto padded = [](const Plan& q, int& hp, int& wp) { hp = std::max(q.H, q.pad_h_to); wp = std::max(q.W, q.pad_w_to); };
    int hp, wp, hpt = 0, wpt = 0;
    padded(p, hp, wp);
    size_t pad_need = (size_t)p.C * hp * wp * es_in, canvas_need = 0;
    if (n_sym > 0) {
        canvas_need = (size_t)p.C * p.out_h * p.out_w * es_out;
        padded(pl_t->p, hpt, wpt);
        pad_need = std::max(pad_need, (size_t)p.C * hpt * wpt * es_in);
    }
    const char* fits = "moe_run_plan_ens: %s of %zu bytes does not fit";
    int rc = n->ens_pad.grow(pad_need, s, fits, "the padded image", pad_need);
    if (!rc && canvas_need) rc = n->ens_canvas.grow(canvas_need, s, fits, "a symmetry's canvas", canvas_need);
    if (rc) return rc;
    rc = sym_pad(img, f16_in, p.C, p.H, p.W, sC, sH, sW, -1, n->ens_pad.p, hp, wp, s);
    if (!rc) rc = moe_run_plan(n, pl, n->ens_pad.p, img_dtype, (int64_t)hp * wp, wp, 1, out, out_dtype, max_tiles, s);
    for (int i = 0; i < n_sym && !rc; ++i) {
        const bool t = sym_of(i).t != 0;
        const int h = t ? hpt : hp, w = t ? wpt : wp;
        rc = sym_pad(img, f16_in, p.C, p.H, p.W, sC, sH, sW, i, n->ens_pad.p, h, w, s);
        if (!rc) rc = moe_run_plan(n, t ? pl_t : pl, n->ens_pad.p, img_dtype, (int64_t)h * w, w, 1, n->ens_canvas.p, out_dtype, max_tiles, s);
        if (!rc) rc = sym_fold(out, n->ens_canvas.p, f16_out, p.C, p.out_h, p.out_w, i, i == n_sym - 1 ? n_sym + 1 : 0, s);
    }
    return rc;
}

extern "C" {

int moe_run_plan_ens(moe_net* n, const moe_plan* pl, const moe_plan* pl_t, int n_sym, const void* img, int img_dtype, int64_t sC, int64_t sH, int64_t sW,
                     void* out, int out_dtype, int max_tiles, void* stream)
{
    if (!n || !pl || !img || !out) return fail(MOE_EINVAL, "moe_run_plan_ens: NULL argument");
    if (n_sym < 0 || n_sym > 7) return fail(MOE_EINVAL, "moe_run_plan_ens: n_sym %d is not in 0..7", n_sym);
    if (!sym_dtype(img_dtype) || !sym_dtype(out_dtype)) return fail(MOE_EINVAL, "moe_run_plan_ens: dtype must be MOE_F32 or MOE_F16");
    const Plan& p = pl->p;
    if (n_sym > 0) {
        if (!pl_t) return fail(MOE_EINVAL, "moe_run_plan_ens: plan_t is NULL (n_sym %d needs the plan of the transposed shape)", n_sym);
        const Plan& q = pl_t->p;
        if (q.C != p.C || q.H != p.W || q.W != p.H || q.sc != p.sc)
            return fail(MOE_EINVAL, "moe_run_plan_ens: plan_t is for %d x %d x %d (scale %d), not the transpose of %d x %d x %d (scale %d)", q.C, q.H, q.W, q.sc, p.C, p.H, p.W, p.sc);
        if (q.out_h != p.out_w || q.out_w != p.out_h)
            return fail(MOE_EINVAL, "moe_run_plan_ens: the two plans disagree on the output shape (%d x %d against %d x %d transposed)", p.out_h, p.out_w, q.out_h, q.out_w);
    }
    if (!n->finalized) return fail(MOE_ESTATE, "moe_run_plan_ens: net is not finalized");
    int prev = -1;
    HIP_TRY(hipGetDevice(&prev));
    HIP_TRY(hipSetDevice(n->device));
    const int rc = run_plan_ens(n, pl, pl_t, n_sym, img, img_dtype, sC, sH, sW, out, out_dtype, max_tiles, (hipStream_t)stream);
    if (prev >= 0 && prev != n->device) (void)hipSetDevice(prev);
    return rc;
}

int moe_to_float(const void* src, int src_dtype, int bits, int H, int W, int C, void* dst, int dst_dtype, int device, void* stream)
{
    if (!src || !dst || H < 1 || W < 1 || C < 1) return fail(MOE_EINVAL, "moe_to_float: bad argument");
    if ((src_dtype != MOE_U8 && src_dtype != MOE_U16) || (dst_dtype != MOE_F32 && dst_dtype != MOE_F16)) return fail(MOE_EINVAL, "moe_to_float: bad dtype");
    HIP_TRY(hipSetDevice(device));
    if (src_dtype == MOE_U8) launch_to_float(src, src_dtype, 255.f, true, H, W, C, dst, dst_dtype, (hipStream_t)stream);
    else launch_to_float(src, src_dtype, 1.f / (float)(1 << bits), false, H, W, C, dst, dst_dtype, (hipStream_t)stream);
    return MOE_OK;
}

int moe_resize(const void* src, void* dst, int dtype, int C, int H, int W, int h, int w, int mode, int device, void* stream)
{
    if (!src || !dst || C < 1 || H < 1 || W < 1 || h < 1 || w < 1) return fail(MOE_EINVAL, "moe_resize: bad argument");
    if (dtype != MOE_F32 && dtype != MOE_F16) return fail(MOE_EINVAL, "moe_resize: dtype must be MOE_F32 or MOE_F16");
    if (mode < MOE_RESIZE_NEAREST || mode > MOE_RESIZE_BICUBIC) return fail(MOE_EINVAL, "moe_resize: unknown mode %d", mode);
    HIP_TRY(hipSetDevice(device));
    launch_resize(src, dst, dtype, C, H, W, h, w, mode, (hipStream_t)stream);
    return launched("resize");
}

int moe_to_output(const void* src, int src_dtype, int H, int W, int C, int bits, void* dst, int dst_dtype, int device, void* stream)
{
    if (!src || !dst || H < 1 || W < 1 || C < 1 || bits < 1 || bits > 16) return fail(MOE_EINVAL, "moe_to_output: bad argument");
    if ((dst_dtype != MOE_U8 && dst_dtype != MOE_U16) || (src_dtype != MOE_F32 && src_dtype != MOE_F16)) return fail(MOE_EINVAL, "moe_to_output: bad dtype");
    if (dst_dtype == MOE_U8 && bits > 8) return fail(MOE_EINVAL, "moe_to_output: %d bits do not fit MOE_U8", bits);
    HIP_TRY(hipSetDevice(device));
    launch_to_output(src, src_dtype, H, W, C, (float)(1 << bits), dst, dst_dtype, (hipStream_t)stream);
    return MOE_OK;
}

int moe_to_yuv(const void* src, int src_dtype, int H, int W, int depth, int matrix, int order, void* dst, int device, void* stream)
{
    if (!src) return fail(MOE_EINVAL, "moe_to_yuv: NULL argument");
    if (H < 1 || W < 1) return fail(MOE_EINVAL, "moe_to_yuv: size %d x %d must be positive", H, W);
    YuvEdge y{};
    const int rc = yuv_edge_args("moe_to_yuv", 3, src_dtype, depth, matrix, order, dst, &y);
    if (rc) return rc;
    y.f16 = 0;
    HIP_TRY(hipSetDevice(device));
    launch_to_output_yuv(src, src_dtype, H, W, y, dst, (hipStream_t)stream);
    return launched("to_output_yuv");
}

}
```

moephoto_amd/csrc/stitch.hip:

```cpp
#include "common.h"
#include <type_traits>
#include "../../include/moephoto_amd.h"

namespace {

__device__ __forceinline__ float stitch_pixel(const StitchArgs& a, int X, int Y, int c)
{
    const int i0 = a.row_first[Y], ni = a.row_cnt[Y];
    const int j0 = a.col_first[X], nj = a.col_cnt[X];
    float cur = 0.f;
    for (int i = max(i0, a.row_lo); i < i0 + ni; ++i) {
        const int fy = a.row_tab[i * 4 + 0], sy = a.row_tab[i * 4 + 1], oy = a.row_tab[i * 4 + 2], eh = a.row_tab[i * 4 + 3];
        for (int j = j0; j < j0 + nj; ++j) {
            const int fx = a.col_tab[j * 4 + 0], sx = a.col_tab[j * 4 + 1], ox = a.col_tab[j * 4 + 2], ew = a.col_tab[j * 4 + 3];
            const float r = a.tiles[a.tile_off[i * a.step_w + j] + ((long long)c * eh + (Y - oy)) * ew + (X - ox)];
            float v1 = r;
            if (Y < sy) v1 = cur + a.ramp[Y - fy] * (r - cur);
            float v = v1;
            if (X < sx) v = cur + a.ramp[X - fx] * (v1 - cur);
            cur = v;
        }
    }
    return cur;
}

struct StitchCols { int j0, ox, ew; };

__device__ __forceinline__ bool stitch_classify(const StitchArgs& a, int X0, StitchCols& k)
{
    if (!(X0 + 8 <= a.out_w)) return false;
    const int j0 = a.col_first[X0], j7 = a.col_first[X0 + 7], n0 = a.col_cnt[X0], n7 = a.col_cnt[X0 + 7];
    const int sx = a.col_tab[j0 * 4 + 1];
    k.j0 = j0; k.ox = a.col_tab[j0 * 4 + 2]; k.ew = a.col_tab[j0 * 4 + 3];
    return (n0 == 1) & (n7 == 1) & (j7 == j0) & (X0 >= sx);
}

template <int NP> struct StitchFold { float v[NP][8]; };

template <int NP>
__device__ __forceinline__ StitchFold<NP> stitch_fold_row(const StitchArgs& a, const StitchCols& k, int X0, int Y, int c0, int np)
{
    StitchFold<NP> f;
    float (&cur)[NP][8] = f.v;
#pragma unroll
    for (int c = 0; c < NP; ++c)
#pragma unroll
        for (int e = 0; e < 8; ++e) cur[c][e] = 0.f;
    const int i0 = a.row_first[Y], ni = a.row_cnt[Y];
    for (int i = max(i0, a.row_lo); i < i0 + ni; ++i) {
        const int fy = a.row_tab[i * 4 + 0], sy = a.row_tab[i * 4 + 1], oy = a.row_tab[i * 4 + 2], eh = a.row_tab[i * 4 + 3];
        const long long plane = (long long)eh * k.ew, o0 = a.tile_off[i * a.step_w + k.j0] + c0 * plane + (long long)(Y - oy) * k.ew + (X0 - k.ox);
        const bool band = Y < sy;
        const float wgt = band ? a.ramp[Y - fy] : 0.f;
#pragma unroll
        for (int c = 0; c < NP; ++c) {
            if (c >= np) break;
            const long long t = o0 + c * plane;
            float q[8];
            if ((t & 3) == 0) {
                const float4 q0 = *(const float4*)(a.tiles + t), q1 = *(const float4*)(a.tiles + t + 4);
                q[0] = q0.x; q[1] = q0.y; q[2] = q0.z; q[3] = q0.w; q[4] = q1.x; q[5] = q1.y; q[6] = q1.z; q[7] = q1.w;
            } else {
#pragma unroll
                for (int e = 0; e < 8; ++e) q[e] = a.tiles[t + e];
            }
            if (band) {
#pragma unroll
                for (int e = 0; e < 8; ++e) cur[c][e] = cur[c][e] + wgt * (q[e] - cur[c][e]);
            } else {
#pragma unroll
                for (int e = 0; e < 8; ++e) cur[c][e] = q[e];
            }
        }
    }
    return f;
}

template <typename T, int N> struct alignas((sizeof(T) * N) % 16 == 0 ? 16 : (sizeof(T) * N) % 8 == 0 ? 8 : 4) StitchRun { T e[N]; };

template <typename T, int N>
__device__ __forceinline__ void stitch_store(T* p, const StitchRun<T, N>& v)
{
    constexpr int A = alignof(StitchRun<T, N>), NV = sizeof(StitchRun<T, N>) / A;
    typedef unsigned vec_t __attribute__((ext_vector_type(A / 4)));
    if (((uintptr_t)p & (A - 1)) == 0) {
        vec_t q[NV];
        __builtin_memcpy(q, &v, sizeof(v));
#pragma unroll
        for (int k = 0; k < NV; ++k) ((vec_t*)p)[k] = q[k];
    } else {
#pragma unroll
        for (int k = 0; k < N; ++k) p[k] = v.e[k];
    }
}

template <int R, typename Edge>
__device__ __forceinline__ void stitch_fold(const StitchArgs& a, const Edge& edge)
{
    __shared__ int s_seam[256];
    __shared__ int s_nseam;
    if (threadIdx.x == 0) s_nseam = 0;
    __syncthreads();
    const int Y0 = blockIdx.y * R + a.y0, yend = a.y0 + a.rows;
    const int X0 = (blockIdx.x * 256 + threadIdx.x) * 8;
    if (X0 < a.out_w) {
        StitchCols k;
        if (!stitch_classify(a, X0, k)) s_seam[atomicAdd(&s_nseam, 1)] = threadIdx.x;
        else {
            typename Edge::Row o[R];
#pragma unroll
            for (int r = 0; r < R; ++r) {
                const int Y = min(Y0 + r, yend - 1);
                const StitchFold<Edge::NP> f = stitch_fold_row<Edge::NP>(a, k, X0, Y, edge.c0(), edge.np(a));
                edge.emit(a, X0, Y, f.v, o[r]);
            }
#pragma unroll
            for (int r = 0; r < R; ++r) {
                if (Y0 + r >= yend) break;
                edge.store(a, X0, Y0 + r, o[r]);
            }
        }
    }
    __syncthreads();
    constexpr int PER = 8 * R * Edge::NOUT;
    const int total = s_nseam * PER;
    for (int t = threadIdx.x; t < total; t += 256) {
        const int gidx = t / PER, rem = t - gidx * PER;
        const int r = rem / (8 * Edge::NOUT), ec = rem - r * (8 * Edge::NOUT);
        const int e = ec / Edge::NOUT, c = ec - e * Edge::NOUT;
        const int X = (blockIdx.x * 256 + s_seam[gidx]) * 8 + e, Y = Y0 + r;
        if (Y >= yend || X >= a.out_w) continue;
        edge.pixel(a, X, Y, c);
    }
}

struct CanvasEdge {
    static constexpr int NP = 1, NOUT = 1;
    struct Row { float v[8]; };
    __device__ __forceinline__ int c0() const { return blockIdx.z; }
    __device__ __forceinline__ int np(const StitchArgs&) const { return 1; }
    __device__ __forceinline__ long long at(const StitchArgs& a, int X, int Y) const { return ((long long)blockIdx.z * a.rows + (Y - a.y0)) * a.out_w + X; }
    __device__ __forceinline__ void emit(const StitchArgs&, int, int, const float (&cur)[1][8], Row& o) const
    {
#pragma unroll
        for (int e = 0; e < 8; ++e) o.v[e] = cur[0][e];
    }
    __device__ __forceinline__ void store(const StitchArgs& a, int X0, int Y, const Row& o) const
    {
        if (a.out_dtype == MOE_F16) {
            StitchRun<half_t, 8> h;
#pragma unroll
            for (int e = 0; e < 8; ++e) h.e[e] = (half_t)o.v[e];
            stitch_store((half_t*)a.out + at(a, X0, Y), h);
        } else {
            StitchRun<float, 8> f;
#pragma unroll
            for (int e = 0; e < 8; ++e) f.e[e] = o.v[e];
            stitch_store((float*)a.out + at(a, X0, Y), f);
        }
    }
    __device__ __forceinline__ void pixel(const StitchArgs& a, int X, int Y, int) const
    {
        const float cur = stitch_pixel(a, X, Y, blockIdx.z);
        if (a.out_dtype == MOE_F16) ((half_t*)a.out)[at(a, X, Y)] = (half_t)cur;
        else ((float*)a.out)[at(a, X, Y)] = cur;
    }
};

template <int R>
__global__ __launch_bounds__(256) void stitch8r_kernel(StitchArgs a)
{
    stitch_fold<R>(a, CanvasEdge());
}

template <typename TD>
__device__ __forceinline__ TD stitch_out_quant(float v, bool f16, float quant)
{
    if (f16) v = (float)(half_t)v;
    v = v * quant;
    v = fminf(fmaxf(v, 0.f), quant - 1.f);
    if (!(v == v)) v = 0.f;
    return (TD)(int)v;
}

template <typename TD, int C>
struct SamplesEdge {
    static constexpr int NP = C, NOUT = C;
    typedef StitchRun<TD, 8 * C> Row;
    float quant; bool f16;
    __device__ __forceinline__ int c0() const { return 0; }
    __device__ __forceinline__ int np(const StitchArgs&) const { return C; }
    __device__ __forceinline__ void emit(const StitchArgs&, int, int, const float (&cur)[C][8], Row& o) const
    {
#pragma unroll
        for (int c = 0; c < C; ++c)
#pragma unroll
            for (int e = 0; e < 8; ++e) o.e[e * C + c] = stitch_out_quant<TD>(cur[c][e], f16, quant);
    }
    __device__ __forceinline__ void store(const StitchArgs& a, int X0, int Y, const Row& o) const { stitch_store((TD*)a.out + ((long long)Y * a.out_w + X0) * C, o); }
    __device__ __forceinline__ void pixel(const StitchArgs& a, int X, int Y, int c) const
    {
        ((TD*)a.out)[((long long)Y * a.out_w + X) * C + c] = stitch_out_quant<TD>(stitch_pixel(a, X, Y, c), f16, quant);
    }
};

template <typename TD, int C, int R>
__global__ __launch_bounds__(256) void stitch_out_kernel(StitchArgs a, float quant, int f16)
{
    stitch_fold<R>(a, SamplesEdge<TD, C>{quant, f16 != 0});
}

template <typename T>
__device__ __forceinline__ T stitch_mix_mul(T h, float f)
{
#pragma clang fp contract(off)
    float p = __fmul_rn(f, (float)h);
    asm("" : "+v"(p));
    return (T)p;
}

__device__ __forceinline__ half_t stitch_mix_mul_once(half_t h, float f)
{
    unsigned r;
    const unsigned hb = __builtin_bit_cast(unsigned short, h);
    const float nz = -0.0f;
    asm("v_fma_mixlo_f16 %0, %1, %2, %3 op_sel_hi:[1,0,0]" : "=v"(r) : "v"(hb), "v"(f), "v"(nz));
    return __builtin_bit_cast(half_t, (unsigned short)(r & 0xffffu));
}
__device__ __forceinline__ float stitch_mix_mul_once(float h, float f) { return stitch_mix_mul<float>(h, f); }

template <typename T>
__device__ __forceinline__ T stitch_mix_value(float cur, T inp, float sf, float tf, bool p_once, bool q_once)
{
#pragma clang fp contract(off)
    const T c = (T)cur;
    const T hp = p_once ? stitch_mix_mul_once(c, sf) : stitch_mix_mul<T>(c, sf);
    const T hq = q_once ? stitch_mix_mul_once(inp, tf) : stitch_mix_mul<T>(inp, tf);
    return (T)__fadd_rn((float)hp, (float)hq);
}

template <typename T>
__device__ __forceinline__ void stitch_mix_load8(const T* p, long long sW, bool vec, T (&v)[8])
{
    if (vec) {
        typedef T vec_t __attribute__((ext_vector_type(16 / sizeof(T))));
        constexpr int N = 16 / sizeof(T);
#pragma unroll
        for (int k = 0; k < 8 / N; ++k) {
            const vec_t q = *(const vec_t*)(p + k * N);
#pragma unroll
            for (int e = 0; e < N; ++e) v[k * N + e] = q[e];
        }
    } else {
#pragma unroll
        for (int e = 0; e < 8; ++e) v[e] = p[e * sW];
    }
}

template <typename T, typename TD, int CT>
struct MixEdge {
    static constexpr bool SAMPLE = !std::is_same<T, TD>::value;
    static constexpr int NP = CT, NOUT = CT;
    struct Planes { StitchRun<T, 8> p[CT]; };
    typedef typename std::conditional<SAMPLE, StitchRun<TD, 8 * CT>, Planes>::type Row;
    const StitchMix& m;
    __device__ __forceinline__ int c0() const { return 0; }
    __device__ __forceinline__ int np(const StitchArgs& a) const { return a.C; }
    __device__ __forceinline__ void emit(const StitchArgs& a, int X0, int Y, const float (&cur)[CT][8], Row& o) const
    {
#pragma unroll
        for (int c = 0; c < CT; ++c) {
            T y[8];
            if (c >= a.C) stitch_mix_load8((const T*)m.alpha + Y * m.aH + X0 * m.aW, m.aW, m.alpha_vec != 0, y);
            else if (m.blend) {
                const long long left = sizeof(T) == 2 ? m.once_from - (((long long)c * a.out_h + Y) * a.out_w + X0) : 8;
                stitch_mix_load8((const T*)m.inp + c * m.sC + Y * m.sH + X0 * m.sW, m.sW, m.inp_vec != 0, y);
#pragma unroll
                for (int e = 0; e < 8; ++e) y[e] = stitch_mix_value<T>(cur[c][e], y[e], m.sf, m.tf, e >= left, e >= left || m.q_once);
            } else {
#pragma unroll
                for (int e = 0; e < 8; ++e) y[e] = (T)cur[c][e];
            }
#pragma unroll
            for (int e = 0; e < 8; ++e) {
                if constexpr (SAMPLE) o.e[e * CT + c] = stitch_out_quant<TD>((float)y[e], false, m.quant);
                else o.p[c].e[e] = y[e];
            }
        }
    }
    __device__ __forceinline__ void store(const StitchArgs& a, int X0, int Y, const Row& o) const
    {
        if constexpr (SAMPLE) stitch_store((TD*)a.out + ((long long)Y * a.out_w + X0) * CT, o);
        else {
#pragma unroll
            for (int c = 0; c < CT; ++c) stitch_store((T*)a.out + ((long long)c * a.out_h + Y) * a.out_w + X0, o.p[c]);
        }
    }
    __device__ __forceinline__ void pixel(const StitchArgs& a, int X, int Y, int c) const
    {
        T y;
        if (c >= a.C) y = ((const T*)m.alpha)[Y * m.aH + X * m.aW];
        else {
            const float cur = stitch_pixel(a, X, Y, c);
            const bool p_once = sizeof(T) == 2 && ((long long)c * a.out_h + Y) * a.out_w + X >= m.once_from;
            y = m.blend ? stitch_mix_value<T>(cur, ((const T*)m.inp)[c * m.sC + Y * m.sH + X * m.sW], m.sf, m.tf, p_once, p_once || m.q_once) : (T)cur;
        }
        if constexpr (SAMPLE) ((TD*)a.out)[((long long)Y * a.out_w + X) * CT + c] = stitch_out_quant<TD>((float)y, false, m.quant);
        else ((T*)a.out)[((long long)c * a.out_h + Y) * a.out_w + X] = y;
    }
};

template <typename T, typename TD, int CT, int R>
__global__ __launch_bounds__(256) void stitch_mix_kernel(StitchArgs a, StitchMix m)
{
    stitch_fold<R>(a, MixEdge<T, TD, CT>{m});
}

__device__ __forceinline__ unsigned yuv_luma(const YuvEdge& y, unsigned p0, unsigned p1, unsigned p2)
{
    const unsigned L = __umul24(y.ky[0], p0) + __umul24(y.ky[1], p1) + __umul24(y.ky[2], p2);
    return y.base_y + (unsigned)(((unsigned long long)L * y.mul_y + 0x80000000ull) >> 32);
}

__device__ __forceinline__ unsigned yuv_chroma(const int (&k)[3], const YuvEdge& y, int s0, int s1, int s2)
{
    const int M = __mul24(k[0], s0) + __mul24(k[1], s1) + __mul24(k[2], s2);
    return (unsigned)(y.base_c + (int)(((long long)M * y.mul_c + 0x80000000ll) >> 32));
}

__device__ __forceinline__ int yuv_sample16(float v, bool f16) { return stitch_out_quant<uint16_t>(v, f16, 65536.f); }

template <typename TD, int R>
__global__ __launch_bounds__(256) void stitch_yuv_kernel(StitchArgs a, YuvEdge y)
{
    static_assert(R % 2 == 0, "a thread owns whole row pairs");
    __shared__ int s_seam[256];
    __shared__ int s_nseam;
    if (threadIdx.x == 0) s_nseam = 0;
    __syncthreads();
    const int Y0 = blockIdx.y * R, X0 = (blockIdx.x * 256 + threadIdx.x) * 8;
    const int cw = (a.out_w + 1) / 2, ch = (a.out_h + 1) / 2;
    TD* const py = (TD*)a.out;
    TD* const pu = py + (long long)a.out_h * a.out_w;
    TD* const pv = pu + (long long)ch * cw;
    const bool f16 = y.f16 != 0;
    if (X0 < a.out_w) {
        StitchCols k;
        if (!stitch_classify(a, X0, k)) s_seam[atomicAdd(&s_nseam, 1)] = threadIdx.x;
        else {
            StitchRun<TD, 8> oy[R];
            StitchRun<TD, 4> ou[R / 2], ov[R / 2];
            int sum[3][4];
#pragma unroll
            for (int r = 0; r < R; ++r) {
                const StitchFold<3> f = stitch_fold_row<3>(a, k, X0, min(Y0 + r, a.out_h - 1), 0, 3);
                int s[3][8];
#pragma unroll
                for (int c = 0; c < 3; ++c)
#pragma unroll
                    for (int e = 0; e < 8; ++e) s[c][e] = yuv_sample16(f.v[c][e], f16);
#pragma unroll
                for (int e = 0; e < 8; ++e) oy[r].e[e] = (TD)yuv_luma(y, s[0][e], s[1][e], s[2][e]);
#pragma unroll
                for (int c = 0; c < 3; ++c)
#pragma unroll
                    for (int e = 0; e < 4; ++e) sum[c][e] = (r & 1 ? sum[c][e] : 0) + s[c][2 * e] + s[c][2 * e + 1];
                if (r & 1) {
#pragma unroll
                    for (int e = 0; e < 4; ++e) {
                        ou[r / 2].e[e] = (TD)yuv_chroma(y.ku, y, sum[0][e], sum[1][e], sum[2][e]);
                        ov[r / 2].e[e] = (TD)yuv_chroma(y.kv, y, sum[0][e], sum[1][e], sum[2][e]);
                    }
                }
            }
#pragma unroll
            for (int r = 0; r < R; ++r) {
                if (Y0 + r >= a.out_h) break;
                stitch_store(py + (long long)(Y0 + r) * a.out_w + X0, oy[r]);
                if (!(r & 1)) {
                    const long long at = (long long)((Y0 + r) / 2) * cw + X0 / 2;
                    stitch_store(pu + at, ou[r / 2]);
                    stitch_store(pv + at, ov[r / 2]);
                }
            }
        }
    }
    __syncthreads();
    constexpr int PER = 4 * (R / 2), NB = 21;
    __shared__ int s_smp[NB * 12];
    const int nblk = s_nseam * PER, t = threadIdx.x;
    auto origin = [&](int b, int& xa, int& ya) {
        const int gidx = b / PER, rem = b - gidx * PER;
        xa = (blockIdx.x * 256 + s_seam[gidx]) * 8 + (rem % 4) * 2; ya = Y0 + (rem / 4) * 2;
        return b < nblk && xa < a.out_w && ya < a.out_h;
    };
    for (int b0 = 0; b0 < nblk; b0 += NB) {
        int xa, ya;
        if (t < NB * 12 && origin(b0 + t / 12, xa, ya)) {
            const int item = t % 12, c = item % 3, i = item / 6, j = (item / 3) & 1;
            const int X = j ? min(xa + 1, a.out_w - 1) : xa, Y = i ? min(ya + 1, a.out_h - 1) : ya;
            s_smp[t] = yuv_sample16(stitch_pixel(a, X, Y, c), f16);
        }
        __syncthreads();
        if (t < NB && origin(b0 + t, xa, ya)) {
            const int* q = s_smp + t * 12;
            int sum[3] = {0, 0, 0};
#pragma unroll
            for (int i = 0; i < 2; ++i)
#pragma unroll
                for (int j = 0; j < 2; ++j) {
                    const int* e = q + (i * 2 + j) * 3;
#pragma unroll
                    for (int c = 0; c < 3; ++c) sum[c] += e[c];
                    if ((i && ya + 1 >= a.out_h) || (j && xa + 1 >= a.out_w)) continue;
                    py[(long long)(ya + i) * a.out_w + xa + j] = (TD)yuv_luma(y, e[0], e[1], e[2]);
                }
            const long long at = (long long)(ya / 2) * cw + xa / 2;
            pu[at] = (TD)yuv_chroma(y.ku, y, sum[0], sum[1], sum[2]);
            pv[at] = (TD)yuv_chroma(y.kv, y, sum[0], sum[1], sum[2]);
        }
        __syncthreads();
    }
}

template <typename TS, typename TD>
__global__ __launch_bounds__(256) void to_output_yuv_kernel(const TS* __restrict__ src, TD* __restrict__ dst, int H, int W, YuvEdge y)
{
    const int X0 = (blockIdx.x * 256 + threadIdx.x) * 8, ya = blockIdx.y * 2;
    if (X0 >= W) return;
    const int cw = (W + 1) / 2, ch = (H + 1) / 2;
    const long long HW = (long long)H * W;
    TD* const pu = dst + HW;
    TD* const pv = pu + (long long)ch * cw;
    const bool whole = X0 + 8 <= W;
    StitchRun<TD, 8> oy[2];
    int sum[3][4];
#pragma unroll
    for (int i = 0; i < 2; ++i) {
        const int Y = min(ya + i, H - 1);
        int s[3][8];
#pragma unroll
        for (int c = 0; c < 3; ++c) {
            const TS* p = src + c * HW + (long long)Y * W;
            TS v[8];
            if (whole) stitch_mix_load8(p + X0, 1, ((uintptr_t)(p + X0) & 15) == 0, v);
            else {
#pragma unroll
                for (int e = 0; e < 8; ++e) v[e] = p[min(X0 + e, W - 1)];
            }
#pragma unroll
            for (int e = 0; e < 8; ++e) s[c][e] = yuv_sample16((float)v[e], false);
#pragma unroll
            for (int e = 0; e < 4; ++e) sum[c][e] = (i ? sum[c][e] : 0) + s[c][2 * e] + s[c][2 * e + 1];
        }
#pragma unroll
        for (int e = 0; e < 8; ++e) oy[i].e[e] = (TD)yuv_luma(y, s[0][e], s[1][e], s[2][e]);
    }
    StitchRun<TD, 4> ou, ov;
#pragma unroll
    for (int e = 0; e < 4; ++e) {
        ou.e[e] = (TD)yuv_chroma(y.ku, y, sum[0][e], sum[1][e], sum[2][e]);
        ov.e[e] = (TD)yuv_chroma(y.kv, y, sum[0][e], sum[1][e], sum[2][e]);
    }
    const long long at = (long long)blockIdx.y * cw + X0 / 2;
    if (whole) {
        stitch_store(dst + (long long)ya * W + X0, oy[0]);
        if (ya + 1 < H) stitch_store(dst + (long long)(ya + 1) * W + X0, oy[1]);
        stitch_store(pu + at, ou);
        stitch_store(pv + at, ov);
    } else {
#pragma unroll
        for (int e = 0; e < 8; ++e) {
            if (X0 + e >= W) break;
            dst[(long long)ya * W + X0 + e] = oy[0].e[e];
            if (ya + 1 < H) dst[(long long)(ya + 1) * W + X0 + e] = oy[1].e[e];
        }
#pragma unroll
        for (int e = 0; e < 4; ++e) {
            if (X0 + 2 * e >= W) break;
            pu[at + e] = ou.e[e]; pv[at + e] = ov.e[e];
        }
    }
}

}

void launch_stitch(const StitchArgs& a, hipStream_t s)
{
    if (a.rows <= 0) return;
    hipLaunchKernelGGL(stitch8r_kernel<4>, dim3(((a.out_w + 7) / 8 + 255) / 256, (a.rows + 3) / 4, a.C), dim3(256), 0, s, a);
}

template <typename TD>
static bool launch_stitch_out_t(const StitchArgs& a, float quant, int f16, hipStream_t s)
{
    constexpr int R = 4;
    const dim3 g(((a.out_w + 7) / 8 + 255) / 256, (a.rows + R - 1) / R);
    if (a.C == 1) hipLaunchKernelGGL((stitch_out_kernel<TD, 1, R>), g, dim3(256), 0, s, a, quant, f16);
    else if (a.C == 2) hipLaunchKernelGGL((stitch_out_kernel<TD, 2, R>), g, dim3(256), 0, s, a, quant, f16);
    else if (a.C == 3) hipLaunchKernelGGL((stitch_out_kernel<TD, 3, R>), g, dim3(256), 0, s, a, quant, f16);
    else if (a.C == 4) hipLaunchKernelGGL((stitch_out_kernel<TD, 4, R>), g, dim3(256), 0, s, a, quant, f16);
    else return false;
    return true;
}

bool launch_stitch_out(const StitchArgs& a, int canvas_dtype, float quant, hipStream_t s)
{
    const int f16 = canvas_dtype == MOE_F16;
    return a.out_dtype == MOE_U8 ? launch_stitch_out_t<uint8_t>(a, quant, f16, s) : launch_stitch_out_t<uint16_t>(a, quant, f16, s);
}

template <typename T, typename TD, int R>
static bool launch_stitch_mix_r(const StitchArgs& a, const StitchMix& m, int planes, hipStream_t s)
{
    const dim3 g(((a.out_w + 7) / 8 + 255) / 256, (a.rows + R - 1) / R);
    if (planes == 1) hipLaunchKernelGGL((stitch_mix_kernel<T, TD, 1, R>), g, dim3(256), 0, s, a, m);
    else if (planes == 2) hipLaunchKernelGGL((stitch_mix_kernel<T, TD, 2, R>), g, dim3(256), 0, s, a, m);
    else if (planes == 3) hipLaunchKernelGGL((stitch_mix_kernel<T, TD, 3, R>), g, dim3(256), 0, s, a, m);
    else if (planes == 4) hipLaunchKernelGGL((stitch_mix_kernel<T, TD, 4, R>), g, dim3(256), 0, s, a, m);
    else return false;
    return true;
}

template <typename T, typename TD>
static bool launch_stitch_mix_t(const StitchArgs& a, const StitchMix& m, int planes, hipStream_t s)
{
    const long long blocks4 = (long long)(((a.out_w + 7) / 8 + 255) / 256) * ((a.out_h + 3) / 4);
    return blocks4 >= 1024 ? launch_stitch_mix_r<T, TD, 4>(a, m, planes, s) : launch_stitch_mix_r<T, TD, 1>(a, m, planes, s);
}

bool launch_stitch_mix(const StitchArgs& a, StitchMix m, int canvas_dtype, hipStream_t s)
{
    const int planes = a.C + (m.alpha ? 1 : 0);
    const bool f16 = canvas_dtype == MOE_F16;
    const long long V = f16 ? 8 : 4;
    m.inp_vec = m.sW == 1 && (uintptr_t)m.inp % 16 == 0 && m.sC % V == 0 && m.sH % V == 0;
    m.alpha_vec = m.alpha && m.aW == 1 && (uintptr_t)m.alpha % 16 == 0 && m.aH % V == 0;
    m.once_from = (long long)a.C * a.out_h * a.out_w / 2048 * 2048;
    m.q_once = f16 && !(m.sW == 1 && (uintptr_t)m.inp % 16 == 0);
    if (m.quant == 0.f) return f16 ? launch_stitch_mix_t<half_t, half_t>(a, m, planes, s) : launch_stitch_mix_t<float, float>(a, m, planes, s);
    if (a.out_dtype == MOE_U8) return f16 ? launch_stitch_mix_t<half_t, uint8_t>(a, m, planes, s) : launch_stitch_mix_t<float, uint8_t>(a, m, planes, s);
    return f16 ? launch_stitch_mix_t<half_t, uint16_t>(a, m, planes, s) : launch_stitch_mix_t<float, uint16_t>(a, m, planes, s);
}

void launch_stitch_yuv(const StitchArgs& a, const YuvEdge& y, hipStream_t s)
{
    constexpr int R = 4;
    const dim3 g(((a.out_w + 7) / 8 + 255) / 256, (a.out_h + R - 1) / R);
    if (y.depth == 8) hipLaunchKernelGGL((stitch_yuv_kernel<uint8_t, R>), g, dim3(256), 0, s, a, y);
    else hipLaunchKernelGGL((stitch_yuv_kernel<uint16_t, R>), g, dim3(256), 0, s, a, y);
}

void launch_to_output_yuv(const void* src, int src_dtype, int H, int W, const YuvEdge& y, void* dst, hipStream_t s)
{
    const dim3 g(((W + 7) / 8 + 255) / 256, (H + 1) / 2);
    if (src_dtype == MOE_F16) {
        if (y.depth == 8) hipLaunchKernelGGL((to_output_yuv_kernel<half_t, uint8_t>), g, dim3(256), 0, s, (const half_t*)src, (uint8_t*)dst, H, W, y);
        else hipLaunchKernelGGL((to_output_yuv_kernel<half_t, uint16_t>), g, dim3(256), 0, s, (const half_t*)src, (uint16_t*)dst, H, W, y);
    } else {
        if (y.depth == 8) hipLaunchKernelGGL((to_output_yuv_kernel<float, uint8_t>), g, dim3(256), 0, s, (const float*)src, (uint8_t*)dst, H, W, y);
        else hipLaunchKernelGGL((to_output_yuv_kernel<float, uint16_t>), g, dim3(256), 0, s, (const float*)src, (uint16_t*)dst, H, W, y);
    }
}
```

Measured before the change: 86.01 MP/s.

## Fold ps4 branch-sum tail into stitch by keeping branch planes

Measured after the change: 86.45 MP/s, median of 6. About the same (+0.5%).

```diff
diff --git a/moephoto_amd/csrc/common.h b/moephoto_amd/csrc/common.h
--- a/moephoto_amd/csrc/common.h
+++ b/moephoto_amd/csrc/common.h
@@ -365,6 +365,7 @@
 
 struct StitchArgs {
     const float* tiles; const long long* tile_off;
+    long long branch; const long long* apron_off;
     const int* row_first; const int* row_cnt;
     const int* col_first; const int* col_cnt;
     const int* row_tab; const int* col_tab;
diff --git a/moephoto_amd/csrc/forward.cpp b/moephoto_amd/csrc/forward.cpp
--- a/moephoto_amd/csrc/forward.cpp
+++ b/moephoto_amd/csrc/forward.cpp
@@ -342,11 +342,23 @@
     return f;
 }
 
-static size_t workspace_need(const moe_net& n, const FwdCtx& ctx, int B, int h, int w)
+static size_t workspace_need(const moe_net& n, const FwdCtx& ctx, int B, int h, int w, bool keep_planes = false)
 {
     Fwd f = make_fwd(n, ctx, nullptr, nullptr, B, h, w, Arena{});
-    run_forward(n, f, FwdIO{});
+    FwdIO io;
+    io.keep_planes = keep_planes;
+    run_forward(n, f, io);
     return f.ar.off + 4096;
+}
+
+long long forward_max_planes(const moe_net& n, int h, int w) { return kSpRange / (sp_bytes_per_pixel(n) * (long long)h * w); }
+
+bool forward_keeps_planes(const moe_net& n, const FwdCtx& ctx, int B, int h, int w)
+{
+    if (!n.finalized || B < 1 || h < 1 || w < 1 || B > forward_max_planes(n, h, w)) return false;
+    if (!(n.arch == MOE_ARCH_NET2X || n.arch == MOE_ARCH_NET3X || n.arch == MOE_ARCH_NET4X)) return false;
+    Fwd f = make_fwd(n, ctx, nullptr, nullptr, B, h, w, Arena{});
+    return arsb_tail_is_ps4(n, f);
 }
 
 static bool plan_matches(const Fwd& f, size_t planned)
@@ -396,11 +408,13 @@
     if (B < 1 || h < 1 || w < 1) return fail(MOE_EINVAL, "moe_net_forward: bad shape B=%d h=%d w=%d", B, h, w);
     if ((io.x_dtype != MOE_F32 && io.x_dtype != MOE_F16) || (io.y_dtype != MOE_F32 && io.y_dtype != MOE_F16))
         return fail(MOE_EINVAL, "moe_net_forward: x/y dtype must be MOE_F32 or MOE_F16");
-    const long long bmax = kSpRange / (sp_bytes_per_pixel(n) * (long long)h * w);
+    const long long bmax = forward_max_planes(n, h, w);
     if (bmax < 1)
         return fail(MOE_ENOMEM, "a %dx%d tile exceeds the convolution kernels' addressing range (%lld pixels per plane at most for this net): use a smaller cropsize",
                     h, w, kSpRange / sp_bytes_per_pixel(n));
     if (n.arch == MOE_ARCH_LITE && io.x_dtype == MOE_F16 && n.lut_state == 0 && n.opt.lite_lut) build_lite_lut(n, s, ctx);
+    if (io.keep_planes && !forward_keeps_planes(n, ctx, B, h, w))
+        return fail(MOE_EINVAL, "internal error: the branch planes of %d planes of %dx%d cannot be kept (not one launch set on conv3x3_ps4's fused tail)", B, h, w);
     if (B <= bmax) return forward_dev_chunk(n, io, B, h, w, s, y_off_mult8, ctx);
     const size_t xe = io.x_dtype == MOE_F32 ? 4 : 2, ye = io.y_dtype == MOE_F32 ? 4 : 2;
     const long long yplane = (long long)h * n.scale * w * n.scale;
@@ -420,7 +434,7 @@
     int cur = -1;
     HIP_TRY(hipGetDevice(&cur));
     if (cur != n.device) HIP_TRY(hipSetDevice(n.device));
-    const size_t need = workspace_need(n, ctx, B, h, w);
+    const size_t need = workspace_need(n, ctx, B, h, w, io.keep_planes);
     StreamSet& set = *ctx.set;
     if (int rc = set.ws.grow(need, s, "workspace of %zu bytes for %d planes of %dx%d does not fit", need, B, h, w)) return rc;
     const size_t planned = need - 4096;
diff --git a/moephoto_amd/csrc/forward_arsb.cpp b/moephoto_amd/csrc/forward_arsb.cpp
--- a/moephoto_amd/csrc/forward_arsb.cpp
+++ b/moephoto_amd/csrc/forward_arsb.cpp
@@ -84,8 +84,11 @@
 template <typename Args, typename Launch>
 int ArsbRun::ps_stage(int br, const std::string& key, const Act& cur, size_t plane_bytes, size_t apron_bytes, const char* name, Launch launch)
 {
-    ps_plane[br] = (float*)f.ar.take(plane_bytes + 4096);
-    ps_apron[br] = (float*)f.ar.take(apron_bytes + 4096);
+    if (f.io.keep_planes) { ps_plane[br] = f.io.plane[br]; ps_apron[br] = f.io.apron[br]; }
+    else {
+        ps_plane[br] = (float*)f.ar.take(plane_bytes + 4096);
+        ps_apron[br] = (float*)f.ar.take(apron_bytes + 4096);
+    }
     if (!f.dry()) {
         const ConvLayer& L = n.convs[n.conv_index.at(key)];
         Args q{};
@@ -235,6 +238,7 @@
 
 int ArsbRun::branch_sum()
 {
+    if (f.io.keep_planes) return MOE_OK;
     if (ps4) { tail_add<TailAddArgs>(launch_tailadd); return MOE_OK; }
     if (ps9) { tail_add<TailAdd3Args>(launch_tailadd3); return MOE_OK; }
     if (fuse) {
@@ -272,6 +276,7 @@
     f.stem(A);
     f.tap("stem", A, h, w, 64, n.C);
     plan_tail_form();
+    if (f.io.keep_planes && !ps4) return fail(MOE_EINVAL, "internal error: %d planes of %dx%d do not end on conv3x3_ps4's fused tail, and their branch planes are to be kept", B, h, w);
     const bool forked = sr && f.ctx.fork && !n.debug && !f.direct && !f.x3 && n.opt.conv_impl == 2 && (long long)B * h * w <= 4ll * 65536;
     struct ForkGuard {
         StreamSet* set; hipStream_t s; bool armed = false;
@@ -323,6 +328,13 @@
 
 }
 
+bool moe::arsb_tail_is_ps4(const moe_net& n, Fwd& f)
+{
+    ArsbRun r{n, f, f.B, f.h, f.w};
+    r.plan_tail_form();
+    return r.ps4;
+}
+
 int moe::forward_arsb(const moe_net& n, Fwd& f)
 {
     ArsbRun r{n, f, f.B, f.h, f.w};
diff --git a/moephoto_amd/csrc/net.h b/moephoto_amd/csrc/net.h
--- a/moephoto_amd/csrc/net.h
+++ b/moephoto_amd/csrc/net.h
@@ -107,6 +107,7 @@
     int calib_log = 0;
     int auto_calibrate = 1;
     int exact_blocks_env = -1;
+    int fold_planes = 1;
     int tiles_per_batch = 0;
     int max_groups = 0;
     int dbg = 0;
@@ -186,6 +187,7 @@
 struct FwdIO {
     const void* x = nullptr; int x_dtype = MOE_F32; long long sB = 0, sH = 0, sW = 0; const long long* x_off = nullptr;
     void* y = nullptr; int y_dtype = MOE_F32; const long long* y_off = nullptr;
+    bool keep_planes = false; float* plane[2] = {nullptr, nullptr}; float* apron[2] = {nullptr, nullptr};
 };
 
 struct FwdCtx {
@@ -326,6 +328,9 @@
 long long sp_bytes_per_pixel(const moe_net& n);
 constexpr long long kSpRange = (1ll << 32) - (1ll << 16);
 int forward_dev(moe_net& n, const FwdIO& io, int B, int h, int w, hipStream_t s, bool y_off_mult8, const FwdCtx& ctx);
+bool forward_keeps_planes(const moe_net& n, const FwdCtx& ctx, int B, int h, int w);
+long long forward_max_planes(const moe_net& n, int h, int w);
+bool arsb_tail_is_ps4(const moe_net& n, Fwd& f);
 void free_set(StreamSet& set);
 void pipe_destroy(moe_net& n);
 void free_records(NetRuntime& rt);
diff --git a/moephoto_amd/csrc/options.cpp b/moephoto_amd/csrc/options.cpp
--- a/moephoto_amd/csrc/options.cpp
+++ b/moephoto_amd/csrc/options.cpp
@@ -59,6 +59,23 @@
     {"repeat", nullptr, kRepeat},
 };
 
+const OptionRow kPlanOptionTable[] = {
+    {"fold_planes", "MOE_FOLD_PLANES", kFlag, &NetOptions::fold_planes},
+};
+
+template <typename F> void each_row(F f)
+{
+    for (const OptionRow& r : kOptionTable) f(r);
+    for (const OptionRow& r : kPlanOptionTable) f(r);
+}
+
+const OptionRow* find_row(const std::string& key)
+{
+    const OptionRow* hit = nullptr;
+    each_row([&](const OptionRow& r) { if (!hit && key == r.key) hit = &r; });
+    return hit;
+}
+
 bool word_value(const OptionWord* words, size_t n, const char* v, int& out)
 {
     for (size_t i = 0; i < n; ++i)
@@ -71,8 +88,8 @@
 bool NetOptions::set(const std::string& key, const char* v)
 {
     if (!v) return false;
-    for (const OptionRow& r : kOptionTable) {
-        if (key != r.key) continue;
+    if (const OptionRow* row = find_row(key)) {
+        const OptionRow& r = *row;
         int t = 0;
         switch (r.kind) {
             case kFlag: if (!word_value(kOnOff, 4, v, t)) return false; break;
@@ -101,9 +118,10 @@
 
 void NetOptions::from_env()
 {
-    for (const OptionRow& r : kOptionTable)
+    each_row([this](const OptionRow& r) {
         if (const char* e = r.env ? getenv(r.env) : nullptr)
             if (!set(r.key, e)) fprintf(stderr, "moephoto_amd: %s=\"%s\" is not a value of option %s -- ignored\n", r.env, e, r.key);
+    });
 
     if (const char* e = getenv("MOE_EXACT_BLOCKS")) exact_blocks_env = atoi(e);
     arsb_trace = getenv("MOE_ARSB_TRACE") != nullptr;
diff --git a/moephoto_amd/csrc/plan_run.cpp b/moephoto_amd/csrc/plan_run.cpp
--- a/moephoto_amd/csrc/plan_run.cpp
+++ b/moephoto_amd/csrc/plan_run.cpp
@@ -28,6 +28,16 @@
     std::vector<std::pair<int, int*>> strip_tabs;
 };
 
+struct PlaneLayout {
+    int device = -1;
+    std::vector<int> per;
+    struct Set { long long plane, apron; };
+    std::vector<Set> sets;
+    long long branch = 0;
+    void* dev = nullptr;
+    const long long *tile_off = nullptr, *apron_off = nullptr;
+};
+
 struct UploadedOffsets { int device; std::vector<int64_t> host; void* dev; };
 
 struct PlanDevice {
@@ -36,12 +46,16 @@
     std::vector<StitchTables> stitch;
     std::vector<UploadedOffsets> uploaded;
     DevBuf pool;
+    DevBuf planes;
+    PlaneLayout fold;
     ~PlanDevice()
     {
         for (auto& t : tables) (void)hipFree(t.dev);
         for (auto& t : stitch) { (void)hipFree(t.dev); for (auto& e : t.strip_tabs) (void)hipFree(e.second); }
         for (auto& u : uploaded) (void)hipFree(u.dev);
+        if (fold.dev) (void)hipFree(fold.dev);
         pool.release();
+        planes.release();
     }
     template <typename V> static int make_room(V& v, hipStream_t s)
     {
@@ -107,24 +121,87 @@
     return MOE_OK;
 }
 
-static int run_sets(moe_net& n, const Plan& p, const TileTable& d, const void* img, int img_dtype, int64_t sH, int64_t sW, float* dst, int max_tiles, hipStream_t s)
+static int tiles_per_set(const moe_net& n, const TileGroup& g, int max_tiles)
 {
     if (max_tiles <= 0) {
         max_tiles = n.opt.tiles_per_batch > 0 ? n.opt.tiles_per_batch : 32;
     }
+    const long long px = (long long)g.th * g.tw;
+    return (int)std::max<long long>(1, (long long)max_tiles * 65536 / std::max<long long>(px, 1));
+}
+
+static int run_sets(moe_net& n, const Plan& p, const TileTable& d, const void* img, int img_dtype, int64_t sH, int64_t sW, float* dst, int max_tiles, hipStream_t s,
+                    const PlaneLayout* keep = nullptr)
+{
+    size_t set = 0;
     for (size_t gi = 0; gi < p.groups.size(); ++gi) {
         const auto& g = p.groups[gi];
         const int nt = d.group_count[gi];
         if (nt < 1) continue;
-        const long long px = (long long)g.th * g.tw;
-        const int per = (int)std::max<long long>(1, std::min<long long>(nt, (long long)max_tiles * 65536 / std::max<long long>(px, 1)));
-        for (int t0 = 0; t0 < nt; t0 += per) {
+        const int per = keep ? keep->per[gi] : std::min(nt, tiles_per_set(n, g, max_tiles));
+        for (int t0 = 0; t0 < nt; t0 += per, ++set) {
             const int cnt = std::min(per, nt - t0);
             const long long slot = (long long)(d.group_first[gi] + t0) * p.C;
-            int rc = forward_dev(n, FwdIO{img, img_dtype, 0, sH, sW, d.x_off + slot, dst, MOE_F32, d.y_off + slot}, cnt * p.C, g.th, g.tw, s, d.y_mult8, own_ctx(n, &n.set));
+            FwdIO io{img, img_dtype, 0, sH, sW, d.x_off + slot, dst, MOE_F32, d.y_off + slot};
+            if (keep) {
+                const PlaneLayout::Set& q = keep->sets[set];
+                io.y = nullptr; io.y_off = nullptr; io.keep_planes = true;
+                for (int br = 0; br < 2; ++br) { io.plane[br] = dst + br * keep->branch + q.plane; io.apron[br] = dst + br * keep->branch + q.apron; }
+            }
+            int rc = forward_dev(n, io, cnt * p.C, g.th, g.tw, s, d.y_mult8, own_ctx(n, &n.set));
             if (rc) return rc;
         }
     }
+    return MOE_OK;
+}
+
+static int plane_layout(moe_net& n, const moe_plan& pl, int max_tiles, hipStream_t s, const PlaneLayout** out)
+{
+    *out = nullptr;
+    const Plan& p = pl.p;
+    if (!n.opt.fold_planes || p.sc < 2 || p.groups.empty()) return MOE_OK;
+    const FwdCtx ctx = own_ctx(n, &n.set);
+    std::vector<int> per;
+    for (const auto& g : p.groups) {
+        const int nt = (int)g.tiles.size();
+        const long long cap = forward_max_planes(n, g.th, g.tw) / p.C;
+        const int k = (int)std::min<long long>(std::min(nt, tiles_per_set(n, g, max_tiles)), cap);
+        if (k < 1 || !forward_keeps_planes(n, ctx, k * p.C, g.th, g.tw) || (nt % k && !forward_keeps_planes(n, ctx, nt % k * p.C, g.th, g.tw))) return MOE_OK;
+        per.push_back(k);
+    }
+    PlaneLayout& L = pl.dev.fold;
+    if (L.dev && L.device == n.device && L.per == per) { *out = &L; return MOE_OK; }
+    if (L.dev) {
+        HIP_TRY(hipStreamSynchronize(s));
+        (void)hipFree(L.dev);
+        L = PlaneLayout{};
+    }
+    const size_t nt = p.tiles.size();
+    std::vector<long long> tab(3 * nt, 0);
+    std::vector<PlaneLayout::Set> sets;
+    long long at = 0;
+    auto take = [&](long long elems) { const long long a = at; at = (at + elems + 1024 + 63) / 64 * 64; return a; };
+    for (size_t gi = 0; gi < p.groups.size(); ++gi) {
+        const auto& g = p.groups[gi];
+        const long long HH = (long long)g.th * p.sc, WW = (long long)g.tw * p.sc, px = (WW + 63) / 64;
+        for (int t0 = 0; t0 < (int)g.tiles.size(); t0 += per[gi]) {
+            const int cnt = std::min(per[gi], (int)g.tiles.size() - t0);
+            const long long B = (long long)cnt * p.C;
+            const PlaneLayout::Set q{take((long long)(ps4_plane_bytes((int)B, (int)HH / 2, (int)WW / 2) / 4)), take((long long)(ps4_apron_bytes((int)B, (int)HH / 2, (int)WW / 2) / 4))};
+            sets.push_back(q);
+            for (int j = 0; j < cnt; ++j) {
+                const size_t k = (size_t)g.tiles[t0 + j];
+                tab[k] = q.plane + (long long)j * p.C * HH * WW;
+                tab[nt + 2 * k] = q.apron + (long long)j * p.C * px * HH;
+                tab[nt + 2 * k + 1] = B * px * HH;
+            }
+        }
+    }
+    int rc = upload(tab.data(), tab.size() * 8, &L.dev);
+    if (rc) return rc;
+    L.device = n.device; L.per = per; L.sets = sets; L.branch = at;
+    L.tile_off = (const long long*)L.dev; L.apron_off = L.tile_off + nt;
+    *out = &L;
     return MOE_OK;
 }
 
@@ -157,7 +234,7 @@
 
 struct OutEdge { int canvas_dtype; float quant; const StitchMix* mix = nullptr; const YuvEdge* yuv = nullptr; };
 static int stitch(const moe_plan& pl, int device, const float* tiles, const int64_t* tile_off, bool off_on_host, int C, void* out, int out_dtype, const int* band, hipStream_t s,
-                  const OutEdge* edge = nullptr)
+                  const OutEdge* edge = nullptr, const PlaneLayout* planes = nullptr)
 {
     const Plan& p = pl.p;
     HIP_TRY(hipSetDevice(device));
@@ -185,6 +262,7 @@
     a.row_tab = d->row_tab; a.col_tab = d->col_tab; a.ramp = d->ramp;
     a.out = out; a.out_dtype = out_dtype; a.C = C; a.out_h = p.out_h; a.out_w = p.out_w; a.step_w = p.aw.step;
     a.y0 = 0; a.rows = p.out_h; a.row_lo = 0;
+    if (planes) { a.tile_off = planes->tile_off; a.branch = planes->branch; a.apron_off = planes->apron_off; }
     if (band) {
         const int row0 = band[0], row1 = band[1], nrow = p.ah.step;
         a.row_lo = row0;
@@ -284,14 +362,24 @@
     const TileTable* d = nullptr;
     int rc = tile_table(*pl, n->device, 0, sC, sH, sW, 1, at.data(), s, &d);
     if (rc) return rc;
-    if (!pool) {
+    const PlaneLayout* keep = nullptr;
+    if (!pool && do_stitch && !edge && shard_count == 1) {
+        rc = plane_layout(*n, *pl, max_tiles, s, &keep);
+        if (rc) return rc;
+    }
+    if (keep) {
+        const size_t bytes = (size_t)keep->branch * 8;
+        rc = pl->dev.planes.grow(bytes, s, "branch planes of %zu bytes do not fit", bytes);
+        if (rc) return rc;
+        pool = (float*)pl->dev.planes.p;
+    } else if (!pool) {
         rc = pl->dev.pool.grow(p.pool_elems_per_plane_set * 4, s, "tile pool of %zu bytes does not fit", p.pool_elems_per_plane_set * 4);
         if (rc) return rc;
         pool = (float*)pl->dev.pool.p;
     }
-    rc = run_sets(*n, p, *d, img, img_dtype, sH, sW, pool, max_tiles, s);
+    rc = run_sets(*n, p, *d, img, img_dtype, sH, sW, pool, max_tiles, s, keep);
     if (rc || !do_stitch) return rc;
-    return stitch(*pl, n->device, pool, nullptr, false, p.C, out, out_dtype, nullptr, s, edge);
+    return stitch(*pl, n->device, pool, nullptr, false, p.C, out, out_dtype, nullptr, s, edge, keep);
 }
 
 extern "C" {
diff --git a/moephoto_amd/csrc/stitch.hip b/moephoto_amd/csrc/stitch.hip
--- a/moephoto_amd/csrc/stitch.hip
+++ b/moephoto_amd/csrc/stitch.hip
@@ -4,6 +4,54 @@
 
 namespace {
 
+__device__ __forceinline__ float stitch_plane_value(const StitchArgs& a, long long t, int k, int cp, int xl, int yl, int eh, int ew)
+{
+    float r = a.tiles[t] + a.tiles[t + a.branch];
+    const int in = xl & 63, col = xl >> 6, px = (ew + 63) >> 6;
+    if (in == 0 && col >= 1) {
+        const long long o = a.apron_off[2 * k] + ((long long)cp * px + (col - 1)) * eh + yl;
+        r += a.tiles[o] + a.tiles[o + a.branch];
+    }
+    if (in == 63 && col + 1 < px) {
+        const long long o = a.apron_off[2 * k] + a.apron_off[2 * k + 1] + ((long long)cp * px + (col + 1)) * eh + yl;
+        r += a.tiles[o] + a.tiles[o + a.branch];
+    }
+    return r;
+}
+
+__device__ __forceinline__ void stitch_plane_row(const StitchArgs& a, long long t, long long ao, long long as, int cp, int xl, int yl, int eh, int ew, float (&q)[8])
+{
+    const int in = xl & 63, col = xl >> 6, px = (ew + 63) >> 6;
+    const int el = (64 - in) & 63, er = 63 - in;
+    const int cl = col + (in != 0);
+    const bool hl = el < 8 && cl >= 1, hr = er < 8 && col + 1 < px;
+    float l0 = 0.f, l1 = 0.f, r0 = 0.f, r1 = 0.f;
+    if (hl) {
+        const float* p = a.tiles + ao + ((long long)cp * px + (cl - 1)) * eh + yl;
+        l0 = p[0]; l1 = p[a.branch];
+    }
+    if (hr) {
+        const float* p = a.tiles + ao + as + ((long long)cp * px + (col + 1)) * eh + yl;
+        r0 = p[0]; r1 = p[a.branch];
+    }
+    const float* p0 = a.tiles + t;
+    const float* p1 = p0 + a.branch;
+    if ((t & 3) == 0) {
+        const float4 v0 = *(const float4*)p0, v1 = *(const float4*)(p0 + 4), u0 = *(const float4*)p1, u1 = *(const float4*)(p1 + 4);
+        q[0] = v0.x + u0.x; q[1] = v0.y + u0.y; q[2] = v0.z + u0.z; q[3] = v0.w + u0.w; q[4] = v1.x + u1.x; q[5] = v1.y + u1.y; q[6] = v1.z + u1.z; q[7] = v1.w + u1.w;
+    } else {
+#pragma unroll
+        for (int e = 0; e < 8; ++e) q[e] = p0[e] + p1[e];
+    }
+    const float sl = l0 + l1, sr = r0 + r1;
+#pragma unroll
+    for (int e = 0; e < 8; ++e) {
+        if (hl && e == el) q[e] = q[e] + sl;
+        if (hr && e == er) q[e] = q[e] + sr;
+    }
+}
+
+template <bool PL = false>
 __device__ __forceinline__ float stitch_pixel(const StitchArgs& a, int X, int Y, int c)
 {
     const int i0 = a.row_first[Y], ni = a.row_cnt[Y];
@@ -13,7 +61,8 @@
         const int fy = a.row_tab[i * 4 + 0], sy = a.row_tab[i * 4 + 1], oy = a.row_tab[i * 4 + 2], eh = a.row_tab[i * 4 + 3];
         for (int j = j0; j < j0 + nj; ++j) {
             const int fx = a.col_tab[j * 4 + 0], sx = a.col_tab[j * 4 + 1], ox = a.col_tab[j * 4 + 2], ew = a.col_tab[j * 4 + 3];
-            const float r = a.tiles[a.tile_off[i * a.step_w + j] + ((long long)c * eh + (Y - oy)) * ew + (X - ox)];
+            const long long t = a.tile_off[i * a.step_w + j] + ((long long)c * eh + (Y - oy)) * ew + (X - ox);
+            const float r = PL ? stitch_plane_value(a, t, i * a.step_w + j, c, X - ox, Y - oy, eh, ew) : a.tiles[t];
             float v1 = r;
             if (Y < sy) v1 = cur + a.ramp[Y - fy] * (r - cur);
             float v = v1;
@@ -37,7 +86,7 @@
 
 template <int NP> struct StitchFold { float v[NP][8]; };
 
-template <int NP>
+template <int NP, bool PL = false>
 __device__ __forceinline__ StitchFold<NP> stitch_fold_row(const StitchArgs& a, const StitchCols& k, int X0, int Y, int c0, int np)
 {
     StitchFold<NP> f;
@@ -52,12 +101,14 @@
         const long long plane = (long long)eh * k.ew, o0 = a.tile_off[i * a.step_w + k.j0] + c0 * plane + (long long)(Y - oy) * k.ew + (X0 - k.ox);
         const bool band = Y < sy;
         const float wgt = band ? a.ramp[Y - fy] : 0.f;
+        const long long ao = PL ? a.apron_off[2 * (i * a.step_w + k.j0)] : 0, as = PL ? a.apron_off[2 * (i * a.step_w + k.j0) + 1] : 0;
 #pragma unroll
         for (int c = 0; c < NP; ++c) {
             if (c >= np) break;
             const long long t = o0 + c * plane;
             float q[8];
-            if ((t & 3) == 0) {
+            if (PL) stitch_plane_row(a, t, ao, as, c0 + c, X0 - k.ox, Y - oy, eh, k.ew, q);
+            else if ((t & 3) == 0) {
                 const float4 q0 = *(const float4*)(a.tiles + t), q1 = *(const float4*)(a.tiles + t + 4);
                 q[0] = q0.x; q[1] = q0.y; q[2] = q0.z; q[3] = q0.w; q[4] = q1.x; q[5] = q1.y; q[6] = q1.z; q[7] = q1.w;
             } else {
@@ -94,7 +145,7 @@
     }
 }
 
-template <int R, typename Edge>
+template <int R, typename Edge, bool PL = false>
 __device__ __forceinline__ void stitch_fold(const StitchArgs& a, const Edge& edge)
 {
     __shared__ int s_seam[256];
@@ -111,7 +162,7 @@
 #pragma unroll
             for (int r = 0; r < R; ++r) {
                 const int Y = min(Y0 + r, yend - 1);
-                const StitchFold<Edge::NP> f = stitch_fold_row<Edge::NP>(a, k, X0, Y, edge.c0(), edge.np(a));
+                const StitchFold<Edge::NP> f = stitch_fold_row<Edge::NP, PL>(a, k, X0, Y, edge.c0(), edge.np(a));
                 edge.emit(a, X0, Y, f.v, o[r]);
             }
 #pragma unroll
@@ -134,6 +185,7 @@
     }
 }
 
+template <bool PL>
 struct CanvasEdge {
     static constexpr int NP = 1, NOUT = 1;
     struct Row { float v[8]; };
@@ -161,7 +213,7 @@
     }
     __device__ __forceinline__ void pixel(const StitchArgs& a, int X, int Y, int) const
     {
-        const float cur = stitch_pixel(a, X, Y, blockIdx.z);
+        const float cur = stitch_pixel<PL>(a, X, Y, blockIdx.z);
         if (a.out_dtype == MOE_F16) ((half_t*)a.out)[at(a, X, Y)] = (half_t)cur;
         else ((float*)a.out)[at(a, X, Y)] = cur;
     }
@@ -170,7 +222,13 @@
 template <int R>
 __global__ __launch_bounds__(256) void stitch8r_kernel(StitchArgs a)
 {
-    stitch_fold<R>(a, CanvasEdge());
+    stitch_fold<R, CanvasEdge<false>, false>(a, CanvasEdge<false>());
+}
+
+template <int R>
+__global__ __launch_bounds__(256) __attribute__((amdgpu_waves_per_eu(8))) void stitch8p_kernel(StitchArgs a)
+{
+    stitch_fold<R, CanvasEdge<true>, true>(a, CanvasEdge<true>());
 }
 
 template <typename TD>
@@ -488,7 +546,9 @@
 void launch_stitch(const StitchArgs& a, hipStream_t s)
 {
     if (a.rows <= 0) return;
-    hipLaunchKernelGGL(stitch8r_kernel<4>, dim3(((a.out_w + 7) / 8 + 255) / 256, (a.rows + 3) / 4, a.C), dim3(256), 0, s, a);
+    const unsigned gx = ((a.out_w + 7) / 8 + 255) / 256;
+    if (a.branch) hipLaunchKernelGGL(stitch8p_kernel<2>, dim3(gx, (a.rows + 1) / 2, a.C), dim3(256), 0, s, a);
+    else hipLaunchKernelGGL(stitch8r_kernel<4>, dim3(gx, (a.rows + 3) / 4, a.C), dim3(256), 0, s, a);
 }
 
 template <typename TD>
```
